# Ham3798/shielded-pool-pinocchio-solana

Measured on AMD Instinct MI355X. Metric: Groth16 proofs/sec, higher is better.
Workload: dtype u32x8 (254-bit Montgomery integers); 1 GPU; audit_circuit (RLWE, const-PK; scripts/generate_audit.py:246-465), batch of 2048 independent proofs per GPU per step, every row a distinct witness; circuit=audit, n_constraints=29178, n_wires=35432, domain=32768, batch_per_gpu=2048, n_distinct_witnesses=2048, table_bytes=223485100032, parallelism=independent proofs x1, pk_bytes=9850060

## Files before the change

shielded-pool-pinocchio-solana_amd/csrc/kernels.hpp:

```cpp
#pragma once
#include <hip/hip_runtime.h>
#include <stdint.h>
#include "bn254.hpp"
#include "msm_plan.hpp"
#include "rlwe_ntt.hpp"

namespace spp {

struct DevSparse {
  const uint32_t* rowptr;
  const uint32_t* wire;
  const uint32_t* coeff;
  const uint32_t* lit;
};
static constexpr uint32_t COEFF_ONE = 0x80000000u;
static constexpr uint32_t COEFF_MINUS_ONE = 0x40000000u;
static constexpr uint32_t COEFF_MASK = 0x3fffffffu;

struct DevCircuit {
  DevSparse A, B, C, H;
  const Fr* coeffs;
  const Fr* aux;
  const uint32_t* program;
  uint32_t n_wires, n_constraints, n_public, n_inputs, challenge_wire;
  const uint32_t* run_start;
  uint32_t n_runs;
  uint32_t max_row_terms;
  const uint8_t* row_flags;
  const uint32_t* sm_wires;
  const int32_t* sm_lo;
  uint32_t sm_nslots;
  const uint32_t* sm_rowptr;
  const uint32_t* sm_slot;
  const int32_t* sm_coef;
  const uint32_t* sm_rest_ptr;
  const uint32_t* sm_rest_wire;
  const uint32_t* sm_rest_coeff;
  const uint32_t* sm_row_out;
  uint32_t sm_nrows;
  const uint8_t* row_small;
  const uint32_t* lg_rows;
  uint32_t lg_n;
  const uint8_t* row_long;
  const Fr* pos3_rc;  const Fr* pos3_mds;
  const Fr* pos5_rc;  const Fr* pos5_mds;
  const Fr* p2_rc;    const Fr* p2_mu;
  const Fr* byte_mont;
  const uint32_t* pos3_mds29;
  const uint32_t* pos5_mds29;
};

struct HashConsts {
  const Fr* pos3_rc;  const Fr* pos3_mds;
  const Fr* pos5_rc;  const Fr* pos5_mds;
  const Fr* p2_rc;    const Fr* p2_mu;
  const uint32_t* pos3_mds29;
  const uint32_t* pos5_mds29;
};

struct RlwePkDev {
  int32_t hat[2][2][1024];
  uint32_t nzeros[2];
  uint16_t zeros[2][1024];
};
struct RlweDev {
  RnTables tb;
  int32_t pk_scale[2];
  RlwePkDev* pk = nullptr;
};
void launch_rlwe_witness(hipStream_t st, const RlweDev& rd, const uint32_t* pk_a, const uint32_t* pk_b, const int8_t* r, const int8_t* e1,
                         const int8_t* e2, const uint8_t* msg, uint32_t* c0, uint32_t* c1, int32_t* k0, int32_t* k1, uint8_t* packed_be,
                         uint32_t count);
void launch_poseidon_hash(hipStream_t st, HashConsts hc, const uint8_t* in_be, uint32_t arity, uint8_t* out_be, uint32_t count);
void launch_merkle_path(hipStream_t st, HashConsts hc, const uint8_t* leaf_be, const uint64_t* index, const uint8_t* siblings_be,
                        uint32_t depth, uint8_t* root_be, uint32_t count);
void launch_merkle_level(hipStream_t st, HashConsts hc, const Fr* children, uint32_t n_children, Fr dflt, Fr* parents, uint32_t n_parents);
struct MerkleTreeDev {
  Fr* level[33];
  uint64_t count[33];
  Fr dflt[33];
  uint32_t depth;
};
void launch_merkle_defaults(hipStream_t st, HashConsts hc, Fr* out, uint32_t depth);
void launch_merkle_update(hipStream_t st, HashConsts hc, const Fr* children, uint64_t n_children, const Fr* dflt_level, Fr* parents,
                          uint64_t first, uint32_t n);
void launch_merkle_gather(hipStream_t st, const MerkleTreeDev* t, uint32_t depth, const uint64_t* indices, uint32_t nq, uint8_t* out_be);
void launch_fr_from_be(hipStream_t st, const uint8_t* in, Fr* out, uint32_t n);
void launch_fr_to_be(hipStream_t st, const Fr* in, uint8_t* out, uint32_t n);
void launch_grumpkin_keygen(hipStream_t st, const GkAffine* table, const uint8_t* sk_be, uint8_t* xy_be, uint32_t count);
void launch_withdraw_rows(hipStream_t st, const GkAffine* table, HashConsts hc, const MerkleTreeDev* t, const uint8_t* notes, uint8_t* rows,
                          uint32_t count);
void launch_deposit_leaves(hipStream_t st, const GkAffine* table, HashConsts hc, const uint8_t* deposits, Fr* leaves, uint32_t count);
void launch_deposit_roots(hipStream_t st, HashConsts hc, const MerkleTreeDev* t, uint64_t first, uint32_t count, uint8_t* roots_be,
                          uint8_t* commitments_be);
void launch_poseidon2_sponge(hipStream_t st, HashConsts hc, const uint8_t* in_be, uint32_t n, uint8_t* out_be, uint32_t count);
void launch_rlwe_decrypt(hipStream_t st, const uint32_t* sk_mod_q, const uint32_t* c0, const uint32_t* c1, uint8_t* msg, uint32_t count);
void launch_shamir_combine(hipStream_t st, const Fr* lambda, const uint8_t* ys_be, uint32_t t, uint32_t n, uint8_t* secret_be,
                           uint32_t* sk_mod_q);
void launch_audit_msg(hipStream_t st, const uint8_t* xy_be, uint8_t* msg, uint32_t count);
void launch_audit_assemble(hipStream_t st, const uint8_t* wa_be, const uint8_t* ct_be, const uint8_t* packed_be, const uint8_t* sk_be,
                           const int8_t* r, const int8_t* e1, const int8_t* e2, const int32_t* k0, const int32_t* k1, uint8_t* rows,
                           uint32_t count);

void launch_load_inputs(hipStream_t st, const uint8_t* d_inputs_be, const uint8_t* d_rs_be, Fr* W, uint32_t n_inputs,
                        uint32_t n_wires, uint32_t P);
static constexpr uint32_t SOLVE_SCRATCH_MIN_ROWS = 324;
void launch_solve(hipStream_t st, DevCircuit dc, Fr* W, Fr* scratch, uint32_t pc_begin, uint32_t pc_end, uint32_t P);
enum : uint32_t { COOP_SEQ = 0, COOP_PAR = 1, COOP_LEVELS = 2, COOP_POSEIDON = 3, COOP_POSEIDON2 = 4, COOP_GRUMPKIN = 5, COOP_LEVEL_STREAM = 6 };
struct DevCoop {
  const uint32_t* items;
  const uint32_t* par;
  const uint32_t* lvl_ptr;
  const uint32_t* lvl_rows;
  const uint32_t* lvl_stream;
};
static constexpr uint32_t COOP_CHUNK = 1024;
static constexpr uint32_t COOP_TRACKS = 4;
struct CoopTracks { uint32_t n; uint32_t begin[COOP_TRACKS], end[COOP_TRACKS]; };
void launch_solve_coop(hipStream_t st, DevCircuit dc, DevCoop co, Fr* W, Fr* scratch, CoopTracks tracks, uint32_t P);
void launch_batch_div(hipStream_t st, DevCircuit dc, Fr* W, Fr* scratch, uint32_t k0, uint32_t n, uint32_t P);
void launch_count8(hipStream_t st, DevCircuit dc, Fr* W, uint32_t* counters, uint32_t h0, uint32_t n, uint32_t out0, uint32_t P);
struct VerifyKeyDev;
void launch_verify(hipStream_t st, const VerifyKeyDev* vk, const uint8_t* proofs, const uint8_t* pws, uint32_t pw_len, uint32_t count,
                   int32_t* ok);
struct PairingCheckDev;
void launch_pairing_check(hipStream_t st, const PairingCheckDev* a, int32_t* ok);
void launch_spmv_check(hipStream_t st, DevCircuit dc, const Fr* W, Fr* abc, uint32_t n, uint32_t P, uint32_t* status, int16_t* small = nullptr);

void launch_ntt(hipStream_t st, Fr* data, uint32_t logn, uint32_t P, const Fr* tw, bool dif, uint32_t nbatch, size_t batch_stride,
                const Fr* post = nullptr);
void launch_scale_rows(hipStream_t st, Fr* data, const Fr* table, uint32_t n, uint32_t P, uint32_t nbatch, size_t batch_stride);
void launch_qap_pointwise(hipStream_t st, Fr* abc, uint32_t n, uint32_t P, Fr zinv);
void launch_qap_product(hipStream_t st, Fr* abc, uint32_t n, uint32_t P);

template <class F>
struct MsmWalk;
template <>
struct MsmWalk<Fq> {
  static constexpr uint32_t waves_per_simd = 2;
  static constexpr bool gather_ahead = false;
};
template <>
struct MsmWalk<Fq2> {
  static constexpr uint32_t waves_per_simd = 1;
  static constexpr bool gather_ahead = true;
};
template <class F>
void launch_build_table(hipStream_t st, const Affine<F>* bases, uint32_t N, uint32_t c, uint32_t Wt, uint32_t row0, uint32_t nrows,
                        Affine<F>* table, XYZZ<F>* tmp, F* tmp_pre);
void launch_msm_digits(hipStream_t st, const uint32_t* rows, const Fr* scalars, int16_t* dig, uint32_t N, uint32_t P, uint32_t c);
template <class F>
void launch_msm_accumulate(hipStream_t st, const Affine<F>* table, const int16_t* dig, XYZZ<F>* partial, uint32_t N, uint32_t P, uint32_t c,
                           const MsmPlan& pl, hipEvent_t ev_start = nullptr, hipEvent_t ev_stop = nullptr);
template <class F>
void launch_msm_reduce(hipStream_t st, XYZZ<F>* partial, XYZZ<F>* out, uint32_t P, const MsmPlan& pl, uint32_t c, bool empty);
static constexpr uint32_t MSM_FOLD_SETS = 8;
static constexpr uint32_t MSM_FOLD_RADIX = 8;
template <class F>
struct MsmFoldSets {
  XYZZ<F>* partial[MSM_FOLD_SETS];
  XYZZ<F>* out[MSM_FOLD_SETS];
  uint32_t Sg[MSM_FOLD_SETS], R[MSM_FOLD_SETS], c[MSM_FOLD_SETS];
  uint32_t cur[MSM_FOLD_SETS], half[MSM_FOLD_SETS];
};
template <class F>
void launch_msm_reduce_multi(hipStream_t st, MsmFoldSets<F> fs, uint32_t nsets, uint32_t P);

void launch_g1_eval_basis(hipStream_t st, const G1Affine* pts, uint32_t n_pts, uint32_t logn, const Fr* scale, const Fr* tw_inv, G1XYZZ* work,
                          G1Affine* out);

void launch_g1_column_sums(hipStream_t st, const G1Affine* base, const uint32_t* row, const Fr* coeff, uint32_t nterms, const uint32_t* seg,
                           uint32_t nseg, G1XYZZ* work, G1Affine* out);

size_t pippenger_workspace_bytes(uint32_t n);
size_t pippenger_workspace_bytes_g2(uint32_t n);
void launch_pippenger_g2(hipStream_t st, const G2Affine* bases, const Fr* scalars, uint32_t n, void* workspace, G2XYZZ** out_windows,
                         hipEvent_t ev0, hipEvent_t ev1);
uint32_t pippenger_windows();
void launch_pippenger_g1(hipStream_t st, const G1Affine* bases, const Fr* scalars, uint32_t n, void* workspace, G1XYZZ** out_windows,
                         hipEvent_t ev0, hipEvent_t ev1);

void launch_challenge(hipStream_t st, const G1XYZZ* commit, Fr* W, uint32_t challenge_wire, uint32_t P, G1Affine* commit_affine,
                      uint32_t* status);
struct AssembleArgs {
  const G1XYZZ* mA; const G1XYZZ* mB1; const G2XYZZ* mB2; const G1XYZZ* mK; const G1XYZZ* mZ; const G1XYZZ* mPok;
  const G1Affine* commit_affine;
  const Fr* W; uint32_t row_r, row_s; uint32_t n_public;
  const G1XYZZ* sAr; const G1XYZZ* rBs1;
  uint8_t* proofs;
  uint8_t* pws;
  uint32_t P;
};
void launch_assemble(hipStream_t st, AssembleArgs a);
void launch_spin(hipStream_t st, uint64_t ticks_100mhz, uint32_t* sink);
void launch_touch(hipStream_t st, uint32_t* sink);
void launch_scale_witness(hipStream_t st, const Fr* W, Fr* Ws, Fr* Wr, uint32_t n_rows, uint32_t row_r, uint32_t row_s, uint32_t P);

template <class F>
void launch_fixed_base_mul(hipStream_t st, const Affine<F>* gen_table, uint32_t c, const Fr* scalars, uint32_t n, Affine<F>* out);

}
```

shielded-pool-pinocchio-solana_amd/csrc/kernels_msm.hip:

```cpp
#include "msm_table.hpp"

namespace spp {

template void launch_build_table<Fq>(hipStream_t, const Affine<Fq>*, uint32_t, uint32_t, uint32_t, uint32_t, uint32_t, Affine<Fq>*,
                                     XYZZ<Fq>*, Fq*);
template void launch_msm_accumulate<Fq>(hipStream_t, const Affine<Fq>*, const int16_t*, XYZZ<Fq>*, uint32_t, uint32_t, uint32_t, const MsmPlan&,
                                        hipEvent_t, hipEvent_t);
template void launch_msm_reduce_multi<Fq>(hipStream_t, MsmFoldSets<Fq>, uint32_t, uint32_t);
template void launch_msm_reduce<Fq>(hipStream_t, XYZZ<Fq>*, XYZZ<Fq>*, uint32_t, const MsmPlan&, uint32_t, bool);
template void launch_fixed_base_mul<Fq>(hipStream_t, const Affine<Fq>*, uint32_t, const Fr*, uint32_t, Affine<Fq>*);

__global__ void __launch_bounds__(256) k_msm_digits(const uint32_t* __restrict__ rows, const Fr* __restrict__ scalars,
                                                    int16_t* __restrict__ dig, uint32_t N, uint32_t P, uint32_t Pp, uint32_t c, uint32_t W) {
  const uint64_t g = (uint64_t)blockIdx.x * blockDim.x + threadIdx.x;
  const uint32_t p = (uint32_t)(g % Pp), i = (uint32_t)(g / Pp);
  if (i >= N || p >= P) return;
  const Fr s = scalars[(size_t)rows[i] * P + p];
  uint32_t l[8];
  s.to_canonical(l);
  const bool neg = canonical_gt_half<FrParams>(l);
  if (neg) {
    uint32_t t[8];
    canonical_negate<FrParams>(l, t);
    SPP_UNROLL for (int k = 0; k < 8; k++) l[k] = t[k];
  }
  const uint32_t mask = (1u << c) - 1u, half = 1u << (c - 1);
  uint32_t carry = 0;
  int16_t* out = dig + (size_t)i * Pp + p;
  const size_t plane = (size_t)N * Pp;
#pragma unroll 1
  for (uint32_t j = 0; j < W; j++) {
    const uint32_t d = (l[0] & mask) + carry;
    SPP_UNROLL for (int k = 0; k < 7; k++) l[k] = (l[k] >> c) | (l[k + 1] << (32 - c));
    l[7] >>= c;
    const bool over = neg ? d > half : d >= half;
    int v = over ? (int)d - (int)(1u << c) : (int)d;
    carry = over ? 1u : 0u;
    if (neg) v = -v;
    out[(size_t)j * plane] = (int16_t)v;
  }
}
void launch_msm_digits(hipStream_t st, const uint32_t* rows, const Fr* scalars, int16_t* dig, uint32_t N, uint32_t P, uint32_t c) {
  if (N == 0 || P == 0) return;
  const uint32_t Pp = msm_padded_batch(P);
  const uint64_t lanes = (uint64_t)N * Pp;
  hipLaunchKernelGGL(k_msm_digits, dim3((uint32_t)((lanes + 255) / 256)), dim3(256), 0, st, rows, scalars, dig, N, P, Pp, c, msm_windows(c));
}

__device__ __forceinline__ XYZZ<Fq> g1_scalar_mul(const XYZZ<Fq>& pt, const Fr& k) {
  uint32_t c[8];
  k.to_canonical(c);
  XYZZ<Fq> acc = XYZZ<Fq>::infinity();
  if (pt.is_inf()) return acc;
#pragma unroll 1
  for (int w = 7; w >= 0; w--) {
    const uint32_t word = w == 0 ? c[0] : w == 1 ? c[1] : w == 2 ? c[2] : w == 3 ? c[3] : w == 4 ? c[4] : w == 5 ? c[5] : w == 6 ? c[6] : c[7];
#pragma unroll 1
    for (int bit = 31; bit >= 0; bit--) {
      acc.dbl_inplace();
      if ((word >> bit) & 1) acc.add(pt);
    }
  }
  return acc;
}
__global__ void __launch_bounds__(64) k_g1_dft_load(const G1Affine* __restrict__ pts, uint32_t n_pts, const Fr* __restrict__ scale,
                                                    G1XYZZ* __restrict__ x, uint32_t n) {
  const uint32_t j = blockIdx.x * blockDim.x + threadIdx.x;
  if (j >= n) return;
  x[j] = j < n_pts ? g1_scalar_mul(G1XYZZ::from_affine(pts[j]), scale[j]) : G1XYZZ::infinity();
}
__global__ void __launch_bounds__(64) k_g1_dft_stage(G1XYZZ* __restrict__ x, uint32_t n, uint32_t len, const Fr* __restrict__ tw) {
  const uint32_t g = blockIdx.x * blockDim.x + threadIdx.x;
  if (g >= n / 2) return;
  const uint32_t half = len / 2, j = g % half, b = (g / half) * len;
  G1XYZZ u = x[b + j], v = x[b + j + half];
  G1XYZZ d = u;
  d.add(v.neg());
  u.add(v);
  x[b + j] = u;
  const uint32_t e = j * (n / len);
  x[b + j + half] = e ? g1_scalar_mul(d, tw[e]) : d;
}
__global__ void __launch_bounds__(64) k_g1_to_affine(const G1XYZZ* __restrict__ x, G1Affine* __restrict__ out, uint32_t n) {
  const uint32_t i = blockIdx.x * blockDim.x + threadIdx.x;
  if (i < n) out[i] = x[i].to_affine();
}
__global__ void __launch_bounds__(64) k_g1_terms(const G1Affine* __restrict__ base, const uint32_t* __restrict__ row, const Fr* __restrict__ coeff,
                                                 uint32_t nterms, G1XYZZ* __restrict__ out) {
  const uint32_t t = blockIdx.x * blockDim.x + threadIdx.x;
  if (t >= nterms) return;
  const G1XYZZ p = G1XYZZ::from_affine(base[row[t]]);
  const Fr c = coeff[t];
  if (c == Fr::one()) out[t] = p;
  else if (c == Fr::one().neg()) out[t] = p.neg();
  else out[t] = g1_scalar_mul(p, c);
}
__global__ void __launch_bounds__(64) k_g1_segsum(const G1XYZZ* __restrict__ terms, const uint32_t* __restrict__ seg, uint32_t nseg,
                                                  G1Affine* __restrict__ out) {
  const uint32_t s = blockIdx.x * blockDim.x + threadIdx.x;
  if (s >= nseg) return;
  G1XYZZ acc = G1XYZZ::infinity();
  for (uint32_t t = seg[s]; t < seg[s + 1]; t++) acc.add(terms[t]);
  out[s] = acc.to_affine();
}
void launch_g1_column_sums(hipStream_t st, const G1Affine* base, const uint32_t* row, const Fr* coeff, uint32_t nterms, const uint32_t* seg,
                           uint32_t nseg, G1XYZZ* work, G1Affine* out) {
  if (nterms) hipLaunchKernelGGL(k_g1_terms, dim3((nterms + 63) / 64), dim3(64), 0, st, base, row, coeff, nterms, work);
  if (nseg) hipLaunchKernelGGL(k_g1_segsum, dim3((nseg + 63) / 64), dim3(64), 0, st, work, seg, nseg, out);
}
void launch_g1_eval_basis(hipStream_t st, const G1Affine* pts, uint32_t n_pts, uint32_t logn, const Fr* scale, const Fr* tw_inv, G1XYZZ* work,
                          G1Affine* out) {
  const uint32_t n = 1u << logn;
  hipLaunchKernelGGL(k_g1_dft_load, dim3((n + 63) / 64), dim3(64), 0, st, pts, n_pts, scale, work, n);
  for (uint32_t len = n; len >= 2; len >>= 1)
    hipLaunchKernelGGL(k_g1_dft_stage, dim3((n / 2 + 63) / 64), dim3(64), 0, st, work, n, len, tw_inv);
  hipLaunchKernelGGL(k_g1_to_affine, dim3((n + 63) / 64), dim3(64), 0, st, work, out, n);
}

}
```

shielded-pool-pinocchio-solana_amd/csrc/kernels_msm_g2.hip:

```cpp
#include "msm_table.hpp"

namespace spp {

template void launch_build_table<Fq2>(hipStream_t, const Affine<Fq2>*, uint32_t, uint32_t, uint32_t, uint32_t, uint32_t, Affine<Fq2>*,
                                      XYZZ<Fq2>*, Fq2*);
template void launch_msm_accumulate<Fq2>(hipStream_t, const Affine<Fq2>*, const int16_t*, XYZZ<Fq2>*, uint32_t, uint32_t, uint32_t,
                                         const MsmPlan&, hipEvent_t, hipEvent_t);
template void launch_msm_reduce_multi<Fq2>(hipStream_t, MsmFoldSets<Fq2>, uint32_t, uint32_t);
template void launch_msm_reduce<Fq2>(hipStream_t, XYZZ<Fq2>*, XYZZ<Fq2>*, uint32_t, const MsmPlan&, uint32_t, bool);
template void launch_fixed_base_mul<Fq2>(hipStream_t, const Affine<Fq2>*, uint32_t, const Fr*, uint32_t, Affine<Fq2>*);

}
```

shielded-pool-pinocchio-solana_amd/csrc/msm_table.hpp:

```cpp
#pragma once
#include <hip/hip_ext.h>
#include "kernels.hpp"
#include <algorithm>
#include "f29.hpp"

namespace spp {

static constexpr unsigned MSM_FOLD_COOP_MAX_BATCH = 8;
static constexpr unsigned MSM_WALK_BLOCK = 64;

template <class F>
__global__ void __launch_bounds__(64) k_build_table(const Affine<F>* __restrict__ bases, uint32_t N, uint32_t c, uint32_t Wn,
                                                    uint32_t step_bits, uint32_t row0, uint32_t nrows, Affine<F>* __restrict__ table,
                                                    XYZZ<F>* __restrict__ tmp, F* __restrict__ tmp_pre) {
  const uint32_t rl = blockIdx.x * blockDim.x + threadIdx.x;
  if (rl >= nrows) return;
  const uint32_t row = row0 + rl;
  const uint32_t E = 1u << (c - 1);
  Affine<F>* out = table + ((size_t)(row >> 6) * E) * 64 + (row & 63);
  XYZZ<F>* t = tmp + rl;
  F* pre = tmp_pre + rl;
  if (row >= N * Wn) {
    for (uint32_t d = 0; d < E; d++) out[(size_t)d * 64] = Affine<F>::infinity();
    return;
  }
  const uint32_t i = row / Wn, j = row % Wn;
  Affine<F> base = bases[i];
  if (base.is_inf()) {
    for (uint32_t d = 0; d < E; d++) out[(size_t)d * 64] = Affine<F>::infinity();
    return;
  }
  XYZZ<F> b = XYZZ<F>::from_affine(base);
  for (uint32_t k = 0; k < step_bits * j; k++) b.dbl_inplace();
  Affine<F> bj = b.to_affine();
  XYZZ<F> acc = XYZZ<F>::from_affine(bj);
  F prod = F::one();
  for (uint32_t d = 0; d < E; d++) {
    t[(size_t)d * nrows] = acc;
    pre[(size_t)d * nrows] = prod;
    prod = prod * (acc.ZZ * acc.ZZZ);
    acc.madd(bj);
  }
  F inv = prod.inv();
  for (uint32_t d = E; d-- > 0;) {
    XYZZ<F> q = t[(size_t)d * nrows];
    F I = inv * pre[(size_t)d * nrows];
    inv = inv * (q.ZZ * q.ZZZ);
    F izz = I * q.ZZZ;
    F izzz = I * q.ZZ;
    out[(size_t)d * 64] = {q.X * izz, q.Y * izzz};
  }
}
template <class F>
void launch_build_table(hipStream_t st, const Affine<F>* bases, uint32_t N, uint32_t c, uint32_t Wt, uint32_t row0, uint32_t nrows,
                        Affine<F>* table, XYZZ<F>* tmp, F* tmp_pre) {
  if (nrows == 0) return;
  const uint32_t W = msm_windows(c);
  if (Wt == 0 || Wt > W) Wt = W;
  const uint32_t R = (W + Wt - 1) / Wt;
  hipLaunchKernelGGL(k_build_table<F>, dim3((nrows + 63) / 64), dim3(64), 0, st, bases, N, c, Wt, c * R, row0, nrows, table, tmp, tmp_pre);
}

struct Recoder {
  uint32_t l[8];
  uint32_t carry;
  bool neg;
  __device__ __forceinline__ void init(const Fr& s) {
    uint32_t cl[8];
    s.to_canonical(cl);
    neg = canonical_gt_half<FrParams>(cl);
    if (neg) {
      canonical_negate<FrParams>(cl, l);
    } else {
      SPP_UNROLL for (int k = 0; k < 8; k++) l[k] = cl[k];
    }
    carry = 0;
  }
  __device__ __forceinline__ uint32_t next(uint32_t c, bool& sgn) {
    const uint32_t mask = (1u << c) - 1u, half = 1u << (c - 1);
    uint32_t d = (l[0] & mask) + carry;
    SPP_UNROLL for (int k = 0; k < 7; k++) l[k] = (l[k] >> c) | (l[k + 1] << (32 - c));
    l[7] >>= c;
    if (d > half) {
      d = (1u << c) - d;
      carry = 1;
      sgn = !neg;
    } else {
      carry = 0;
      sgn = neg;
    }
    return d;
  }
};

__device__ __forceinline__ bool words_all_zero(const Fq& v) {
  uint32_t o = 0;
  SPP_UNROLL for (int i = 0; i < 8; i++) o |= v.l[i];
  return o == 0;
}
template <class F>
struct MsmAcc;
template <>
struct MsmAcc<Fq> {
  XYZZ29<FqParams> a;
  __device__ __forceinline__ void init() { a = XYZZ29<FqParams>::infinity(); }
  __device__ __forceinline__ void madd(const Affine<Fq>& e, bool sgn) {
    if (words_all_zero(e.x) && words_all_zero(e.y)) return;
    a.madd(e, sgn);
  }
  __device__ __forceinline__ XYZZ<Fq> result() const { return a.to_xyzz(); }
};

template <>
struct MsmAcc<Fq2> {
  XYZZ29G2 a;
  __device__ __forceinline__ void init() { a = XYZZ29G2::infinity(); }
  __device__ __forceinline__ void madd(const Affine<Fq2>& e, bool sgn) {
    if (words_all_zero(e.x.c0) && words_all_zero(e.x.c1) && words_all_zero(e.y.c0) && words_all_zero(e.y.c1)) return;
    a.madd(e, sgn);
  }
  __device__ __forceinline__ XYZZ<Fq2> result() const { return a.to_xyzz(); }
};


template <class F>
__global__ void __launch_bounds__(MSM_WALK_BLOCK, MsmWalk<F>::waves_per_simd) k_msm_flat(const Affine<F>* __restrict__ table, const int16_t* __restrict__ dig,
                                                  XYZZ<F>* __restrict__ partial, uint32_t N, uint32_t P, uint32_t Pp, uint32_t c,
                                                  uint32_t R, uint32_t Sg) {
  const uint32_t g = blockIdx.x * blockDim.x + threadIdx.x;
  const uint32_t p = g % Pp, t = g / Pp;
  if (t >= R * Sg || p >= P) return;
  const uint32_t rho = t / Sg, sl = t % Sg;
  const uint32_t E = 1u << (c - 1);
  const int16_t* __restrict__ dg = dig + ((size_t)rho * N) * Pp + p;
  MsmAcc<F> acc;
  acc.init();
  if constexpr (MsmWalk<F>::gather_ahead) {
    int d_next = 0;
    Affine<F> e_next;
    for (uint32_t i0 = sl;; i0 += 4 * Sg) {
      const bool last = i0 >= N;
      uint64_t pack = 0;
      if (!last) {
        SPP_UNROLL for (uint32_t k = 0; k < 4; k++) {
          const uint32_t i = i0 + k * Sg;
          const uint32_t d = i < N ? (uint32_t)(uint16_t)dg[(size_t)i * Pp] : 0u;
          pack |= (uint64_t)d << (16 * k);
        }
      }
#pragma unroll 1
      for (uint32_t k = 0; k < 4; k++) {
        const int d = (int)(int16_t)(uint16_t)(pack >> (16 * k));
        const bool flush = last && k == 0;
        if (d != 0 || flush) {
          Affine<F> e;
          if (d != 0) {
            const uint32_t i = i0 + k * Sg;
            const uint32_t mag = (uint32_t)(d < 0 ? -d : d);
            e = table[((size_t)(i >> 6) * E + (mag - 1)) * 64 + (i & 63)];
          }
          if (d_next != 0) acc.madd(e_next, d_next < 0);
          d_next = d;
          if (d != 0) e_next = e;
        }
      }
      if (last) break;
    }
  } else {
    for (uint32_t i0 = sl; i0 < N; i0 += 4 * Sg) {
      uint64_t pack = 0;
      SPP_UNROLL for (uint32_t k = 0; k < 4; k++) {
        const uint32_t i = i0 + k * Sg;
        const uint32_t d = i < N ? (uint32_t)(uint16_t)dg[(size_t)i * Pp] : 0u;
        pack |= (uint64_t)d << (16 * k);
      }
      if (pack == 0) continue;
#pragma unroll 1
      for (uint32_t k = 0; k < 4; k++) {
        const int d = (int)(int16_t)(uint16_t)(pack >> (16 * k));
        if (d != 0) {
          const uint32_t i = i0 + k * Sg;
          const uint32_t mag = (uint32_t)(d < 0 ? -d : d);
          acc.madd(table[((size_t)(i >> 6) * E + (mag - 1)) * 64 + (i & 63)], d < 0);
        }
      }
    }
  }
  partial[(size_t)t * P + p] = acc.result();
}

template <class F>
__global__ void __launch_bounds__(256) k_msm_rows(const Affine<F>* __restrict__ table, const int16_t* __restrict__ dig,
                                                  XYZZ<F>* __restrict__ partial, uint32_t N, uint32_t P, uint32_t Pp, uint32_t c,
                                                  uint32_t Wt, uint32_t R, uint32_t W, uint32_t Sg, uint32_t Q, uint32_t Wq) {
  const uint32_t g = blockIdx.x * blockDim.x + threadIdx.x;
  const uint32_t p = g % Pp, t = g / Pp;
  if (t >= R * Sg || p >= P) return;
  const uint32_t rho = t / Sg, sl = t % Sg;
  const uint32_t E = 1u << (c - 1);
  const size_t plane = (size_t)N * Pp;
  MsmAcc<F> acc;
  acc.init();
  const uint32_t items = N * Q;
  for (uint32_t it = sl; it < items; it += Sg) {
    uint32_t i = it, q = 0;
    if (Q > 1) {
      i = it % N;
      q = it / N;
    }
    const uint32_t m0 = q * Wq, m1 = m0 + Wq < Wt ? m0 + Wq : Wt;
    const int16_t* __restrict__ dg = dig + (size_t)i * Pp + p;
#pragma unroll 1
    for (uint32_t m = m0; m < m1; m++) {
      const uint32_t j = rho + R * m;
      if (j >= W) break;
      const int d = dg[(size_t)j * plane];
      if (d != 0) {
        const uint32_t row = i * Wt + m;
        const uint32_t mag = (uint32_t)(d < 0 ? -d : d);
        acc.madd(table[((size_t)(row >> 6) * E + (mag - 1)) * 64 + (row & 63)], d < 0);
      }
    }
  }
  partial[(size_t)t * P + p] = acc.result();
}

template <class F>
void launch_msm_accumulate(hipStream_t st, const Affine<F>* table, const int16_t* dig, XYZZ<F>* partial, uint32_t N, uint32_t P, uint32_t c,
                           const MsmPlan& pl, hipEvent_t ev_start, hipEvent_t ev_stop) {
  if (N == 0 || P == 0) {
    if (ev_start) hipEventRecord(ev_start, st);
    if (ev_stop) hipEventRecord(ev_stop, st);
    return;
  }
  const uint64_t lanes = (uint64_t)pl.R * pl.Sg * pl.Pp;
  if (pl.Wt == 1)
    hipExtLaunchKernelGGL(k_msm_flat<F>, dim3((uint32_t)((lanes + MSM_WALK_BLOCK - 1) / MSM_WALK_BLOCK)), dim3(MSM_WALK_BLOCK), 0, st, ev_start, ev_stop, 0, table, dig, partial, N, P, pl.Pp, c, pl.R, pl.Sg);
  else
    hipExtLaunchKernelGGL(k_msm_rows<F>, dim3((uint32_t)((lanes + 255) / 256)), dim3(256), 0, st, ev_start, ev_stop, 0, table, dig, partial, N, P, pl.Pp, c,
                          pl.Wt, pl.R, pl.W, pl.Sg, pl.Q, pl.Wq);
}

template <class T>
__device__ __forceinline__ T msm_shfl_xor(const T& v, int mask) {
  static_assert(sizeof(T) % 4 == 0, "word-sized");
  T r;
  const uint32_t* s = reinterpret_cast<const uint32_t*>(&v);
  uint32_t* d = reinterpret_cast<uint32_t*>(&r);
  SPP_UNROLL for (uint32_t i = 0; i < sizeof(T) / 4; i++) d[i] = (uint32_t)__shfl_xor((int)s[i], mask, 64);
  return r;
}
template <class F>
__global__ void __launch_bounds__(64) k_msm_fold_multi(MsmFoldSets<F> fs, uint32_t P, uint32_t coop) {
  const uint32_t set = blockIdx.y, rho = blockIdx.z;
  const uint32_t next = fs.half[set], S_cur = fs.cur[set];
  if (next == 0 || rho >= fs.R[set]) return;
  const uint32_t g = blockIdx.x * blockDim.x + threadIdx.x;
  XYZZ<F>* __restrict__ partial = fs.partial[set] + (size_t)rho * fs.Sg[set] * P;
  if (coop) {
    static_assert(MSM_FOLD_RADIX == 8, "three shuffle steps");
    const uint32_t o = g >> 3, m = g & 7;
    const bool live = o < next * P;
    const uint32_t s = live ? o / P : 0, p = live ? o % P : 0, t = s + next * m;
    XYZZ<F> a = XYZZ<F>::infinity();
    if (live && t < S_cur) a = partial[(size_t)t * P + p];
    SPP_UNROLL for (int d = 4; d >= 1; d >>= 1) {
      const XYZZ<F> b = msm_shfl_xor(a, d);
      a.add(b);
    }
    if (live && m == 0) {
      if (next == 1 && fs.R[set] == 1) fs.out[set][p] = a;
      else partial[(size_t)s * P + p] = a;
    }
    return;
  }
  if (g >= next * P) return;
  const uint32_t s = g / P, p = g % P;
  XYZZ<F> a = partial[(size_t)s * P + p];
#pragma unroll 1
  for (uint32_t t = s + next; t < S_cur; t += next) a.add(partial[(size_t)t * P + p]);
  if (next == 1 && fs.R[set] == 1) fs.out[set][p] = a;
  else partial[(size_t)s * P + p] = a;
}
template <class F>
__global__ void __launch_bounds__(64) k_msm_horner(MsmFoldSets<F> fs, uint32_t P) {
  const uint32_t set = blockIdx.y;
  const uint32_t R = fs.R[set], c = fs.c[set];
  const uint32_t p = blockIdx.x * blockDim.x + threadIdx.x;
  if (R <= 1 || p >= P) return;
  const size_t stride = (size_t)fs.Sg[set] * P;
  const XYZZ<F>* __restrict__ sums = fs.partial[set];
  XYZZ<F> acc = sums[(size_t)(R - 1) * stride + p];
#pragma unroll 1
  for (uint32_t rho = R - 1; rho-- > 0;) {
    if (!acc.is_inf()) {
      F X = acc.X * acc.ZZ, Y = acc.Y * acc.ZZZ, Z = acc.ZZ;
#pragma unroll 1
      for (uint32_t k = 0; k < c; k++) {
        const F A = X.sqr(), B = Y.sqr(), C = B.sqr();
        const F t = (X + B).sqr() - A - C;
        const F D = t.dbl();
        const F E = A.dbl() + A;
        const F X3 = E.sqr() - D.dbl();
        const F C8 = C.dbl().dbl().dbl();
        const F Z3 = (Y * Z).dbl();
        Y = E * (D - X3) - C8;
        X = X3;
        Z = Z3;
      }
      const F zz = Z.sqr();
      acc.X = X;
      acc.Y = Y;
      acc.ZZ = zz;
      acc.ZZZ = zz * Z;
    }
    acc.add(sums[(size_t)rho * stride + p]);
  }
  fs.out[set][p] = acc;
}
template <class F>
__global__ void __launch_bounds__(256) k_msm_fill_inf(XYZZ<F>* __restrict__ out, uint32_t P) {
  const uint32_t g = blockIdx.x * blockDim.x + threadIdx.x;
  if (g < P) out[g] = XYZZ<F>::infinity();
}

template <class F>
void launch_msm_reduce_multi(hipStream_t st, MsmFoldSets<F> fs, uint32_t nsets, uint32_t P) {
  if (P == 0 || nsets == 0) return;
  uint32_t cur[MSM_FOLD_SETS];
  bool done[MSM_FOLD_SETS];
  uint32_t maxR = 1;
  bool horner = false;
  for (uint32_t i = 0; i < nsets; i++) {
    cur[i] = fs.Sg[i];
    done[i] = false;
    if (fs.Sg[i] == 0) {
      hipLaunchKernelGGL(k_msm_fill_inf<F>, dim3((P + 255) / 256), dim3(256), 0, st, fs.out[i], P);
      done[i] = true;
      fs.R[i] = 1;
      continue;
    }
    if (fs.R[i] > 1) horner = true;
    if (fs.R[i] > 1 && fs.Sg[i] == 1) done[i] = true;
    maxR = std::max(maxR, fs.R[i]);
  }
  for (;;) {
    uint64_t lanes = 0;
    for (uint32_t i = 0; i < nsets; i++) {
      fs.half[i] = done[i] ? 0 : (cur[i] + MSM_FOLD_RADIX - 1) / MSM_FOLD_RADIX;
      fs.cur[i] = cur[i];
      lanes = std::max<uint64_t>(lanes, (uint64_t)fs.half[i] * P);
    }
    if (lanes == 0) break;
    const uint32_t coop = P <= MSM_FOLD_COOP_MAX_BATCH ? 1u : 0u;
    if (coop) lanes *= MSM_FOLD_RADIX;
    hipLaunchKernelGGL(k_msm_fold_multi<F>, dim3((uint32_t)((lanes + 63) / 64), nsets, maxR), dim3(64), 0, st, fs, P, coop);
    for (uint32_t i = 0; i < nsets; i++)
      if (!done[i]) {
        cur[i] = fs.half[i];
        if (cur[i] == 1) done[i] = true;
      }
  }
  if (horner) {
    for (uint32_t i = 0; i < nsets; i++)
      if (fs.Sg[i] == 0) fs.R[i] = 1;
    hipLaunchKernelGGL(k_msm_horner<F>, dim3((P + 63) / 64, nsets), dim3(64), 0, st, fs, P);
  }
}
template <class F>
void launch_msm_reduce(hipStream_t st, XYZZ<F>* partial, XYZZ<F>* out, uint32_t P, const MsmPlan& pl, uint32_t c, bool empty) {
  MsmFoldSets<F> fs{};
  fs.partial[0] = partial;
  fs.out[0] = out;
  fs.Sg[0] = empty ? 0 : pl.Sg;
  fs.R[0] = pl.R;
  fs.c[0] = c;
  launch_msm_reduce_multi<F>(st, fs, 1, P);
}

template <class F>
__global__ void __launch_bounds__(64) k_fixed_base_mul(const Affine<F>* __restrict__ gen_table, uint32_t c, uint32_t Wn,
                                                       const Fr* __restrict__ scalars, uint32_t n, Affine<F>* __restrict__ out) {
  const uint32_t i = blockIdx.x * blockDim.x + threadIdx.x;
  if (i >= n) return;
  const uint32_t E = 1u << (c - 1);
  Fr s = scalars[i];
  XYZZ<F> acc = XYZZ<F>::infinity();
  if (!s.is_zero()) {
    Recoder rc;
    rc.init(s);
#pragma unroll 1
    for (uint32_t j = 0; j < Wn; j++) {
      bool sgn;
      uint32_t d = rc.next(c, sgn);
      if (d != 0) {
        Affine<F> e = gen_table[((size_t)(j >> 6) * E + (d - 1)) * 64 + (j & 63)];
        if (sgn) e.y = e.y.neg();
        acc.madd(e);
      }
    }
  }
  out[i] = acc.to_affine();
}
template <class F>
void launch_fixed_base_mul(hipStream_t st, const Affine<F>* gen_table, uint32_t c, const Fr* scalars, uint32_t n, Affine<F>* out) {
  if (n == 0) return;
  hipLaunchKernelGGL(k_fixed_base_mul<F>, dim3((n + 63) / 64), dim3(64), 0, st, gen_table, c, msm_windows(c), scalars, n, out);
}

}
```

shielded-pool-pinocchio-solana_amd/csrc/spp_circuit.hpp:

```cpp
#pragma once
#include "spp_internal.hpp"

template <class F>
struct MsmSet {
  uint32_t N = 0;
  Affine<F>* table = nullptr;
  uint32_t* rows = nullptr;
  bool from_h = false;
  uint32_t c = 0;
  uint32_t Wt = 0;
};
template <class F>
struct MsmBuf {
  XYZZ<F>* partial = nullptr;
  XYZZ<F>* out = nullptr;
  size_t partial_cap = 0;
  MsmPlan plan{};
};
struct Workspace {
  hipStream_t st = nullptr;
  hipStream_t st2 = nullptr;
  hipStream_t own_st = nullptr, own_st2 = nullptr;
  hipStream_t own_st2p = nullptr;
  std::pair<hipEvent_t, hipEvent_t> g2_ev{nullptr, nullptr};
  hipEvent_t ev_w = nullptr, ev_b2 = nullptr;
  hipEvent_t ev_in = nullptr, ev_rows = nullptr;
  size_t cap = 0, last_P = 0;
  Fr *W = nullptr, *abc = nullptr, *scratch = nullptr;
  G1Affine* commit_affine = nullptr;
  uint8_t *d_inputs = nullptr, *d_rs = nullptr, *d_proofs = nullptr, *d_pws = nullptr;
  uint32_t* d_status = nullptr;
  uint32_t* counters = nullptr;
  MsmBuf<Fq> A, B1, K, Z, CB, CS;
  MsmBuf<Fq> sA, rB;
  Fr *Ws = nullptr, *Wr = nullptr;
  MsmBuf<Fq2> B2;
  int16_t *dig1 = nullptr, *dig2 = nullptr;
  size_t dig1_cap = 0, dig2_cap = 0;
  int16_t* small = nullptr;
  void* audit_scratch = nullptr;
  size_t audit_scratch_cap = 0;
  std::vector<void*> owned;
  hipEvent_t ev[8] = {};
  std::vector<std::pair<hipEvent_t, hipEvent_t>> msm_ev;
  size_t msm_ev_used = 0;
};

template <class F>
struct PendingTable {
  std::vector<Affine<F>> pts;
  Affine<F>* table;
  uint32_t c, Wt;
};
struct SolveStep {
  enum Kind { SEQ, BATCH_DIV, COUNT8, COMMIT } kind;
  uint32_t a = 0, b = 0, c = 0;
  uint32_t ntracks = 0, tr_begin[COOP_TRACKS] = {}, tr_end[COOP_TRACKS] = {};
};
struct Switches {
  int h_mode = 2;
  bool no_coop = false;
  bool trace_items = false;
  bool one_track = false;
  bool no_level_stream = false;
  uint32_t coop_max_batch = 1024;
  bool no_side = false;
  int forced_depth = 0;
  bool no_split = false;
  MsmTuning msm;
};
static constexpr uint64_t SCALED_BLIND_MAX_SCALARS = 1500000;
inline uint32_t scaled_blind_max_batch(uint32_t n_a, uint32_t n_b1) {
  const uint64_t n = (uint64_t)n_a + n_b1;
  return n ? (uint32_t)std::max<uint64_t>(1, std::min<uint64_t>(1024, SCALED_BLIND_MAX_SCALARS / n)) : 1;
}
struct spp_circuit {
  spp_ctx* ctx = nullptr;
  std::vector<SolveStep> schedule;
  Circuit circ;
  DevCircuit dc{};
  uint32_t c_bits = 10, n = 0, logn = 0;
  uint32_t max_batch_div = SOLVE_SCRATCH_MIN_ROWS;
  DevCoop coop{};
  Switches sw;
  bool generic_solver = false;
  uint32_t row_r = 0, row_s = 0, row_rs = 0, n_rows = 0;
  size_t in_stride = 0, pw_stride = 0;
  uint64_t table_bytes = 0;
  MsmSet<Fq> A, B1, K, Z, CB, CS;
  MsmSet<Fq2> B2;
  Fr *tw_fwd = nullptr, *tw_inv = nullptr, *coset_br = nullptr, *coset_inv_br = nullptr;
  Fr zinv;
  std::vector<void*> owned;
  Workspace ws[SPP_NWS];
  int next_ws = 0, last_ws = 0, prev_ws = 0;
  std::vector<PendingTable<Fq>> pending1;
  std::vector<PendingTable<Fq2>> pending2;
};

template <class T>
static int own_upload(spp_circuit* c, T** dst, const std::vector<T>& src) {
  HIP_TRY(dev_upload(dst, src));
  c->owned.push_back((void*)*dst);
  return 0;
}

#pragma GCC visibility push(hidden)
int coop_plan(spp_circuit* c);
int row_paths_plan(spp_circuit* c);
void destroy_circuit(spp_circuit* c);
void free_workspace(Workspace& w);
#pragma GCC visibility pop
```

shielded-pool-pinocchio-solana_amd/csrc/spp_load.cpp:

```cpp
#include "spp_circuit.hpp"

static std::vector<PendingTable<Fq>>& pending(spp_circuit* c, Fq*) { return c->pending1; }
static std::vector<PendingTable<Fq2>>& pending(spp_circuit* c, Fq2*) { return c->pending2; }

static int upload_sparse(spp_circuit* c, const Circuit& circ, const Sparse& m, DevSparse* out) {
  std::vector<uint32_t> wire(m.terms.size()), coeff(m.terms.size()), lit(m.terms.size(), 0);
  Fr one = Fr::one(), mone = Fr::one().neg();
  std::vector<uint32_t> small(circ.coeffs.size(), 0);
  for (size_t ci = 0; ci < circ.coeffs.size(); ci++) {
    uint32_t v[8], nv[8];
    circ.coeffs[ci].to_canonical(v);
    bool hi0 = true;
    for (int k = 1; k < 8; k++) hi0 = hi0 && v[k] == 0;
    if (hi0 && v[0] != 0 && v[0] < (1u << 28)) { small[ci] = v[0]; continue; }
    circ.coeffs[ci].neg().to_canonical(nv);
    hi0 = true;
    for (int k = 1; k < 8; k++) hi0 = hi0 && nv[k] == 0;
    if (hi0 && nv[0] != 0 && nv[0] < (1u << 28)) small[ci] = nv[0] | 0x80000000u;
  }
  for (size_t i = 0; i < m.terms.size(); i++) {
    wire[i] = m.terms[i].wire;
    uint32_t ci = m.terms[i].coeff;
    uint32_t flag = 0;
    if (circ.coeffs[ci] == one) flag = COEFF_ONE;
    else if (circ.coeffs[ci] == mone) flag = COEFF_MINUS_ONE;
    else lit[i] = small[ci];
    coeff[i] = ci | flag;
  }
  uint32_t *rp, *w, *co, *li;
  if (int e = own_upload(c, &li, lit)) return e;
  out->lit = li;
  if (int e = own_upload(c, &rp, m.rowptr)) return e;
  if (int e = own_upload(c, &w, wire)) return e;
  if (int e = own_upload(c, &co, coeff)) return e;
  out->rowptr = rp;
  out->wire = w;
  out->coeff = co;
  return 0;
}

template <class F>
static int alloc_table(spp_circuit* c, size_t N, uint32_t cbits, uint32_t Wt, Affine<F>** table_out) {
  size_t table_elems = std::max<size_t>(msm_table_elems((uint32_t)N, cbits, Wt), 1);
  Affine<F>* table;
  HIP_TRY(hipMalloc((void**)&table, table_elems * sizeof(Affine<F>)));
  c->owned.push_back(table);
  c->table_bytes += table_elems * sizeof(Affine<F>);
  *table_out = table;
  return 0;
}
template <class F>
static int build_table(spp_circuit* c, const std::vector<Affine<F>>& pts, uint32_t cbits, uint32_t Wt, Affine<F>* table, size_t temp_budget) {
  hipStream_t st = c->ctx->stream;
  const uint32_t Wn = Wt, E = 1u << (cbits - 1);
  const size_t N = pts.size();
  if (N == 0) return 0;
  const size_t rows_total = msm_table_rows(N, Wn);
  const size_t per_row = (size_t)E * (sizeof(XYZZ<F>) + sizeof(F));
  size_t chunk = std::max<size_t>(64, ((temp_budget / per_row) / 64) * 64);
  chunk = std::min(chunk, (size_t)65536);
  chunk = std::min(chunk, rows_total);
  DevBuf d_bases, tmp, tmp_pre;
  HIP_TRY(d_bases.alloc(N * sizeof(Affine<F>)));
  HIP_TRY(hipMemcpy(d_bases.p, pts.data(), N * sizeof(Affine<F>), hipMemcpyHostToDevice));
  HIP_TRY(tmp.alloc(chunk * E * sizeof(XYZZ<F>)));
  HIP_TRY(tmp_pre.alloc(chunk * E * sizeof(F)));
  for (size_t r0 = 0; r0 < rows_total; r0 += chunk) {
    uint32_t cnt = (uint32_t)std::min(chunk, rows_total - r0);
    launch_build_table<F>(st, d_bases.as<Affine<F>>(), (uint32_t)N, cbits, Wt, (uint32_t)r0, cnt, table, tmp.as<XYZZ<F>>(), tmp_pre.as<F>());
  }
  HIP_TRY(hipStreamSynchronize(st));
  HIP_TRY(hipGetLastError());
  return 0;
}
static size_t table_temp_budget() {
  size_t free_b = 0, total_b = 0;
  if (hipMemGetInfo(&free_b, &total_b) != hipSuccess) return (size_t)2 << 30;
  size_t b = free_b / 2;
  b = std::min(b, (size_t)48 << 30);
  return std::max(b, (size_t)1 << 28);
}
template <class F>
static int build_table_chunked(spp_circuit* c, const std::vector<Affine<F>>& pts, uint32_t cbits, uint32_t Wt, Affine<F>** table_out) {
  if (int e = alloc_table<F>(c, pts.size(), cbits, Wt, table_out)) return e;
  return build_table<F>(c, pts, cbits, Wt, *table_out, std::min(table_temp_budget(), (size_t)2 << 30));
}


template <class F>
static int make_set(spp_circuit* c, MsmSet<F>* set, const std::vector<uint32_t>& rows, const std::vector<Affine<F>>& pts, bool from_h,
                    uint32_t cbits, bool flat) {
  set->N = (uint32_t)pts.size();
  set->from_h = from_h;
  set->c = cbits;
  set->Wt = flat ? 1 : msm_windows(cbits);
  if (int e = own_upload(c, &set->rows, rows)) return e;
  if (int e = alloc_table<F>(c, pts.size(), cbits, set->Wt, &set->table)) return e;
  pending(c, (F*)nullptr).push_back({pts, set->table, cbits, set->Wt});
  return 0;
}
static int build_pending(spp_circuit* c) {
  const size_t budget = table_temp_budget();
  int e = 0;
  for (auto& p : pending(c, (Fq*)nullptr)) if (!e) e = build_table<Fq>(c, p.pts, p.c, p.Wt, p.table, budget);
  for (auto& p : pending(c, (Fq2*)nullptr)) if (!e) e = build_table<Fq2>(c, p.pts, p.c, p.Wt, p.table, budget);
  pending(c, (Fq*)nullptr).clear();
  pending(c, (Fq2*)nullptr).clear();
  return e;
}

namespace {
struct PkFile {
  uint32_t circuit_id, n_wires, domain_log, n_public, challenge_wire;
  G1Affine alpha1, beta1, delta1;
  G2Affine beta2, delta2;
  std::vector<uint32_t> A_w, B1_w, B2_w, K_w, CB_w, CS_w;
  std::vector<G1Affine> A, B1, K, Z, CB, CS;
  std::vector<G2Affine> B2;
};
struct Rd {
  const uint8_t* p;
  const uint8_t* end;
  bool ok = true;
  uint32_t u32() {
    if (p + 4 > end) { ok = false; return 0; }
    uint32_t v = (uint32_t)p[0] | ((uint32_t)p[1] << 8) | ((uint32_t)p[2] << 16) | ((uint32_t)p[3] << 24);
    p += 4;
    return v;
  }
  const uint8_t* take(size_t n) {
    if (p + n > end) { ok = false; return nullptr; }
    const uint8_t* q = p;
    p += n;
    return q;
  }
};
bool rd_g1_section(Rd& r, std::vector<uint32_t>* wires, std::vector<G1Affine>& pts) {
  uint32_t n = r.u32();
  if (!r.ok || (size_t)n * 64 > (size_t)(r.end - r.p)) return false;
  if (wires) {
    wires->resize(n);
    for (auto& w : *wires) w = r.u32();
  }
  pts.resize(n);
  for (auto& pt : pts) {
    const uint8_t* b = r.take(64);
    if (!b) return false;
    pt = g1_from_raw(b);
  }
  return r.ok;
}
bool parse_pk(const std::vector<uint8_t>& buf, PkFile& k) {
  Rd r{buf.data(), buf.data() + buf.size()};
  if (r.u32() != 0x4b505053u || r.u32() != 1) return false;
  k.circuit_id = r.u32(); k.n_wires = r.u32(); k.domain_log = r.u32(); k.n_public = r.u32(); k.challenge_wire = r.u32();
  const uint8_t* b;
  if (!(b = r.take(64))) return false; k.alpha1 = g1_from_raw(b);
  if (!(b = r.take(64))) return false; k.beta1 = g1_from_raw(b);
  if (!(b = r.take(64))) return false; k.delta1 = g1_from_raw(b);
  if (!(b = r.take(128))) return false; k.beta2 = g2_from_raw(b);
  if (!(b = r.take(128))) return false; k.delta2 = g2_from_raw(b);
  if (!rd_g1_section(r, &k.A_w, k.A)) return false;
  if (!rd_g1_section(r, &k.B1_w, k.B1)) return false;
  uint32_t n2 = r.u32();
  if (!r.ok || (size_t)n2 * 128 > (size_t)(r.end - r.p)) return false;
  k.B2_w.resize(n2);
  for (auto& w : k.B2_w) w = r.u32();
  k.B2.resize(n2);
  for (auto& pt : k.B2) {
    if (!(b = r.take(128))) return false;
    pt = g2_from_raw(b);
  }
  if (!rd_g1_section(r, &k.K_w, k.K)) return false;
  if (!rd_g1_section(r, nullptr, k.Z)) return false;
  if (!rd_g1_section(r, &k.CB_w, k.CB)) return false;
  if (!rd_g1_section(r, &k.CS_w, k.CS)) return false;
  return r.ok && r.p == r.end;
}
}


template <class F>
static void merge_point(std::vector<uint32_t>& wires, std::vector<Affine<F>>& pts, uint32_t wire, const Affine<F>& extra) {
  for (size_t i = 0; i < wires.size(); i++)
    if (wires[i] == wire) {
      pts[i] = host_add(pts[i], extra);
      return;
    }
  wires.push_back(wire);
  pts.push_back(extra);
}

namespace {
struct PlanSet {
  double n, esz, wgt;
  bool flat;
  int bits;
};
double plan_bytes(const PlanSet& s, int cb) { return s.n * s.esz * (s.flat ? 1.0 : (double)msm_windows((uint32_t)cb)) * (double)(1u << (cb - 1)); }
void plan_greedy(std::vector<PlanSet>& sets, double budget, int cmax) {
  double used = 0;
  for (auto& s : sets) used += plan_bytes(s, s.bits);
  for (;;) {
    int best = -1;
    double best_gain = 0;
    for (size_t i = 0; i < sets.size(); i++) {
      const PlanSet& s = sets[i];
      if (s.wgt == 0 || s.bits >= cmax || s.n == 0) continue;
      const double extra = plan_bytes(s, s.bits + 1) - plan_bytes(s, s.bits);
      if (used + extra > budget) continue;
      const double saved = s.wgt * s.n * ((double)msm_windows((uint32_t)s.bits) - (double)msm_windows((uint32_t)s.bits + 1));
      double gain = saved / extra;
      if (saved <= 0) gain = 1e-30;
      if (gain > best_gain) { best_gain = gain; best = (int)i; }
    }
    if (best < 0) break;
    used += plan_bytes(sets[best], sets[best].bits + 1) - plan_bytes(sets[best], sets[best].bits);
    sets[best].bits++;
  }
}
const double PLAN_ESZ[7] = {64, 64, 64, 64, 64, 64, 128}, PLAN_WGT[7] = {1, 1, 1, 1, 0, 0, 3.0};
}

struct LoadState {
  PkFile pk;
  uint32_t cw[7];
  bool flat[7] = {false, false, false, false, false, false, false};
  std::vector<uint32_t> z_w, xk_w;
  std::vector<G1Affine> z_p, xk_p;
};

static Switches read_switches() {
  Switches sw;
  const char* hm = getenv("SPP_H_MODE");
  sw.h_mode = hm ? atoi(hm) : (getenv("SPP_Z_COEFF") ? 0 : 2);
  if (sw.h_mode < 0 || sw.h_mode > 2) sw.h_mode = 2;
  sw.no_coop = getenv("SPP_NO_COOP") != nullptr;
  sw.trace_items = getenv("SPP_COOP_TRACE") != nullptr;
  sw.one_track = getenv("SPP_COOP_ONE_TRACK") != nullptr;
  sw.no_level_stream = getenv("SPP_NO_LEVEL_STREAM") != nullptr;
  if (const char* e = getenv("SPP_COOP_MAX")) sw.coop_max_batch = (uint32_t)atoi(e);
  sw.no_side = getenv("SPP_NO_SIDE") != nullptr;
  const char* de = getenv("SPP_DEPTH");
  const int depth = de ? atoi(de) : 0;
  sw.forced_depth = depth >= 1 && depth <= SPP_NWS ? depth : 0;
  sw.no_split = getenv("SPP_NO_SPLIT") != nullptr;
  sw.msm = msm_tuning_from_env(getenv("SPP_MSM_WAVES"), getenv("SPP_MSM_WAVES_SMALL"));
  return sw;
}

static int plan_load_windows(const PkFile& pk, int window_bits, const uint32_t* forced_bits, uint32_t cw[7], bool flat[7]) {
  const double nset[7] = {(double)pk.A.size() + 2, (double)pk.B1.size() + 2, (double)pk.K.size() + 1, (double)pk.Z.size(),
                          (double)pk.CB.size(), (double)pk.CS.size(), (double)pk.B2.size() + 2};
  if (forced_bits) {
    for (int s = 0; s < 7; s++) {
      cw[s] = forced_bits[s];
      flat[s] = PLAN_WGT[s] != 0;
    }
  } else if (window_bits != 0) {
    for (int s = 0; s < 7; s++) cw[s] = (uint32_t)window_bits;
  } else {
    const char* fe = getenv("SPP_FLAT");
    const bool use_flat = !(fe && fe[0] == '0');
    size_t free_b = 0, total_b = 0;
    HIP_TRY(hipMemGetInfo(&free_b, &total_b));
    double budget = 240e9;
    if (const char* env = getenv("SPP_TABLE_BUDGET_GB")) budget = atof(env) * 1e9;
    budget = std::min(budget, 0.85 * (double)free_b);
    std::vector<PlanSet> sets;
    for (int s = 0; s < 7; s++) {
      flat[s] = use_flat && PLAN_WGT[s] != 0;
      sets.push_back({nset[s], PLAN_ESZ[s], PLAN_WGT[s], flat[s], PLAN_WGT[s] != 0 ? 6 : 9});
    }
    plan_greedy(sets, budget, use_flat ? 16 : 15);
    for (int s = 0; s < 7; s++) cw[s] = (uint32_t)sets[s].bits;
  }
  return 0;
}

static int load_r1cs(spp_circuit* c) {
  const Circuit& circ = c->circ;
  int e;
  if ((e = upload_sparse(c, circ, circ.A, &c->dc.A)) || (e = upload_sparse(c, circ, circ.B, &c->dc.B)) ||
      (e = upload_sparse(c, circ, circ.C, &c->dc.C)) || (e = upload_sparse(c, circ, circ.H, &c->dc.H)))
    return e;
  Fr* d_coeffs;
  Fr* d_aux;
  uint32_t* d_prog;
  if ((e = own_upload(c, &d_coeffs, circ.coeffs)) || (e = own_upload(c, &d_prog, circ.program)) || (e = own_upload(c, &d_aux, circ.aux))) return e;
  c->dc.coeffs = d_coeffs;
  c->dc.aux = d_aux;
  c->dc.program = d_prog;
  c->dc.n_wires = circ.n_wires;
  c->dc.n_constraints = circ.n_constraints;
  {
    std::vector<uint32_t> runs;
    auto same_b = [&](uint32_t k) {
      const uint32_t a0 = circ.B.rowptr[k - 1], a1 = circ.B.rowptr[k], b1 = circ.B.rowptr[k + 1];
      if (a1 - a0 != b1 - a1 || a1 == a0) return false;
      for (uint32_t t = 0; t < a1 - a0; t++)
        if (circ.B.terms[a0 + t].wire != circ.B.terms[a1 + t].wire || circ.B.terms[a0 + t].coeff != circ.B.terms[a1 + t].coeff) return false;
      return true;
    };
    uint32_t len = 0;
    for (uint32_t k = 0; k < circ.n_constraints; k++) {
      if (k == 0 || len >= 8 || !same_b(k)) { runs.push_back(k); len = 0; }
      len++;
    }
    const uint32_t n_runs = (uint32_t)runs.size();
    runs.push_back(circ.n_constraints);
    uint32_t* d_runs;
    if ((e = own_upload(c, &d_runs, runs))) return e;
    c->dc.run_start = d_runs;
    c->dc.n_runs = n_runs;
    uint32_t longest = 0;
    for (const Sparse* m : {&circ.A, &circ.B, &circ.C})
      for (uint32_t k = 0; k < circ.n_constraints; k++) longest = std::max(longest, m->rowptr[k + 1] - m->rowptr[k]);
    c->dc.max_row_terms = longest;
    std::vector<uint8_t> flags(std::max<uint32_t>(circ.n_constraints, 1), 0);
    for (uint32_t k = 0; k < circ.n_constraints; k++) {
      if (k > 0 && same_b(k)) flags[k] |= 1;
      const uint32_t a0 = circ.A.rowptr[k], a1 = circ.A.rowptr[k + 1], b0 = circ.B.rowptr[k], b1 = circ.B.rowptr[k + 1];
      bool eq = a1 - a0 == b1 - b0 && a1 != a0;
      for (uint32_t t = 0; eq && t < a1 - a0; t++)
        eq = circ.A.terms[a0 + t].wire == circ.B.terms[b0 + t].wire && circ.A.terms[a0 + t].coeff == circ.B.terms[b0 + t].coeff;
      if (eq) flags[k] |= 2;
    }
    uint8_t* d_flags;
    if ((e = own_upload(c, &d_flags, flags))) return e;
    c->dc.row_flags = d_flags;
  }
  c->dc.n_public = circ.n_public;
  c->dc.n_inputs = circ.n_inputs();
  c->dc.challenge_wire = circ.challenge_wire;
  {
    auto flat = [](const PoseidonParams& pp) {
      std::vector<Fr> m;
      for (auto& row : pp.mds)
        for (auto& v : row) m.push_back(v);
      return m;
    };
    const PoseidonParams& p3 = poseidon_params(3);
    const PoseidonParams& p5 = poseidon_params(5);
    const Poseidon2Params& p2 = poseidon2_params();
    Fr *a, *b, *cc, *d, *f, *g;
    std::vector<Fr> mu(p2.mu, p2.mu + 4);
    auto canon = [](std::vector<Fr> v) {
      for (auto& x : v) x = x.canonical();
      return v;
    };
    if ((e = own_upload(c, &a, canon(p3.rc))) || (e = own_upload(c, &b, flat(p3))) || (e = own_upload(c, &cc, canon(p5.rc))) ||
        (e = own_upload(c, &d, flat(p5))) || (e = own_upload(c, &f, p2.rc)) || (e = own_upload(c, &g, mu)))
      return e;
    std::vector<Fr> bytes(256);
    for (int i = 0; i < 256; i++) bytes[i] = Fr::from_u64((uint64_t)i);
    Fr* bm;
    if ((e = own_upload(c, &bm, bytes))) return e;
    c->dc.byte_mont = bm;
    auto flat29 = [](const PoseidonParams& pp) {
      std::vector<uint32_t> m;
      for (auto& row : pp.mds)
        for (auto& v : row) {
          const F29<FrParams> x = F29<FrParams>::from_fp(v);
          for (int k = 0; k < 9; k++) m.push_back(x.l[k]);
        }
      return m;
    };
    uint32_t *m3, *m5;
    if ((e = own_upload(c, &m3, flat29(p3))) || (e = own_upload(c, &m5, flat29(p5)))) return e;
    c->dc.pos3_mds29 = m3;
    c->dc.pos5_mds29 = m5;
    c->dc.pos3_rc = a; c->dc.pos3_mds = b; c->dc.pos5_rc = cc; c->dc.pos5_mds = d; c->dc.p2_rc = f; c->dc.p2_mu = g;
  }
  return 0;
}

static int load_program(spp_circuit* c) {
  const Circuit& circ = c->circ;
  bool generic_ops = false;
  {
    const auto& pr = circ.program;
    size_t pc = 0, seg = 0;
    auto flush = [&](size_t end) {
      if (end > seg) c->schedule.push_back({SolveStep::SEQ, (uint32_t)seg, (uint32_t)end, 0});
    };
    const bool trace_ops = getenv("SPP_SOLVE_TRACE") != nullptr;
    if (trace_ops) c->sw.no_coop = true;
    uint32_t prev_op = OP_END;
    while (pc < pr.size() && pr[pc] != OP_END) {
      if (trace_ops && pr[pc] != prev_op) {
        flush(pc);
        seg = std::max(seg, pc);
      }
      prev_op = pr[pc];
      switch (pr[pc]) {
        case OP_SOLVE_C: case OP_SOLVE_A: case OP_MASK: pc += 2; break;
        case OP_BATCH_DIV:
          c->max_batch_div = std::max(c->max_batch_div, pr[pc + 2]);
          if (pr[pc + 2] >= 64) {
            flush(pc);
            c->schedule.push_back({SolveStep::BATCH_DIV, pr[pc + 1], pr[pc + 2], 0});
            seg = pc + 3;
          }
          pc += 3;
          break;
        case OP_COUNT8:
          flush(pc);
          c->schedule.push_back({SolveStep::COUNT8, pr[pc + 1], pr[pc + 2], pr[pc + 3]});
          seg = pc + 4;
          pc += 4;
          break;
        case OP_BITS: case OP_LIMBS8: case OP_POSEIDON: pc += 4; break;
        case OP_POSEIDON2: case OP_INV_H: pc += 3; break;
        case OP_COMMIT:
          flush(pc);
          c->schedule.push_back({SolveStep::COMMIT, 0, 0, 0});
          pc += 1;
          seg = pc;
          break;
        case OP_GRUMPKIN: pc += 5 + pr[pc + 4]; break;
        case OP_SOLVE_ROW: case OP_LIMBS: case OP_COUNTN: pc += 5; generic_ops = true; break;
        case OP_GK_MUL: pc += 7; generic_ops = true; break;
        case OP_GLV: pc += 3 + 28; generic_ops = true; break;
        case OP_EMUL: pc += 3 + 16; generic_ops = true; break;
        default: return fail(SPP_ERR_FORMAT, "bad opcode %u in solver program", pr[pc]);
      }
    }
    flush(pc);
  }

  c->generic_solver = generic_ops;
  if (generic_ops) c->sw.no_coop = true;
  else if (int e = coop_plan(c)) return e;
  if (int e = row_paths_plan(c)) return e;
  return 0;
}

static int load_ntt_tables(spp_circuit* c) {
  int e;
  const uint32_t n = c->n, logn = c->logn;
  Fr w = fr_root_of_unity(logn), wi = w.inv();
  std::vector<Fr> tf(n / 2), ti(n / 2), cb(n), cib(n);
  Fr a = Fr::one(), b = Fr::one();
  for (uint32_t k = 0; k < n / 2; k++) {
    tf[k] = a;
    ti[k] = b;
    a = a * w;
    b = b * wi;
  }
  Fr g = c->sw.h_mode == 2 ? fr_root_of_unity(logn + 1) : Fr::from_u64(5), gi = g.inv(), ninv = Fr::from_u64(n).inv();
  std::vector<Fr> gp(n), gip(n);
  Fr x = ninv, y = ninv;
  for (uint32_t i = 0; i < n; i++) {
    gp[i] = x;
    gip[i] = y;
    x = x * g;
    y = y * gi;
  }
  for (uint32_t pos = 0; pos < n; pos++) {
    uint32_t i = bitrev(pos, logn);
    cb[pos] = gp[i];
    cib[pos] = gip[i];
  }
  if ((e = own_upload(c, &c->tw_fwd, tf)) || (e = own_upload(c, &c->tw_inv, ti)) || (e = own_upload(c, &c->coset_br, cb)) ||
      (e = own_upload(c, &c->coset_inv_br, cib)))
    return e;
  Fr gn = g.pow_u64(n);
  c->zinv = (gn - Fr::one()).inv();
  return 0;
}

static int load_key_sets(spp_circuit* c, const LoadState& s) {
  const PkFile& pk = s.pk;
  const uint32_t* cw = s.cw;
  const bool* flat = s.flat;
  int e;
  {
    std::vector<uint32_t> w = pk.A_w;
    std::vector<G1Affine> p = pk.A;
    merge_point(w, p, 0u, pk.alpha1);
    w.push_back(c->row_r); p.push_back(pk.delta1);
    if ((e = make_set(c, &c->A, w, p, false, cw[0], flat[0]))) return e;
  }
  {
    std::vector<uint32_t> w = pk.B1_w;
    std::vector<G1Affine> p = pk.B1;
    merge_point(w, p, 0u, pk.beta1);
    w.push_back(c->row_s); p.push_back(pk.delta1);
    if ((e = make_set(c, &c->B1, w, p, false, cw[1], flat[1]))) return e;
  }
  {
    std::vector<uint32_t> w = pk.B2_w;
    std::vector<G2Affine> p = pk.B2;
    merge_point(w, p, 0u, pk.beta2);
    w.push_back(c->row_s); p.push_back(pk.delta2);
    if ((e = make_set(c, &c->B2, w, p, false, cw[6], flat[6]))) return e;
  }
  return 0;
}

static int load_h_bases(spp_circuit* c, LoadState& s) {
  const PkFile& pk = s.pk;
  const Circuit& circ = c->circ;
  spp_ctx* ctx = c->ctx;
  std::vector<uint32_t>&z_w = s.z_w, &xk_w = s.xk_w;
  std::vector<G1Affine>&z_p = s.z_p, &xk_p = s.xk_p;
  int e;
  if (pk.Z.size() != (size_t)c->n - 1) return fail(SPP_ERR_FORMAT, "Z section has %zu points, expected %u", pk.Z.size(), c->n - 1);
  const uint32_t n = c->n;
  hipStream_t st = ctx->stream;
  auto eval_basis = [&](const std::vector<Fr>& scale, std::vector<G1Affine>& out) -> int {
    DevBuf d_pts, d_scale, d_work, d_out;
    HIP_TRY(d_pts.alloc(pk.Z.size() * sizeof(G1Affine)));
    HIP_TRY(d_scale.alloc((size_t)n * sizeof(Fr)));
    HIP_TRY(d_work.alloc((size_t)n * sizeof(G1XYZZ)));
    HIP_TRY(d_out.alloc((size_t)n * sizeof(G1Affine)));
    HIP_TRY(hipMemcpyAsync(d_pts.p, pk.Z.data(), pk.Z.size() * sizeof(G1Affine), hipMemcpyHostToDevice, st));
    HIP_TRY(hipMemcpyAsync(d_scale.p, scale.data(), (size_t)n * sizeof(Fr), hipMemcpyHostToDevice, st));
    launch_g1_eval_basis(st, d_pts.as<G1Affine>(), (uint32_t)pk.Z.size(), c->logn, d_scale.as<Fr>(), c->tw_inv, d_work.as<G1XYZZ>(),
                         d_out.as<G1Affine>());
    std::vector<G1Affine> br(n);
    HIP_TRY(hipMemcpyAsync(br.data(), d_out.p, (size_t)n * sizeof(G1Affine), hipMemcpyDeviceToHost, st));
    HIP_TRY(hipStreamSynchronize(st));
    HIP_TRY(hipGetLastError());
    out.resize(n);
    for (uint32_t pos = 0; pos < n; pos++) out[bitrev(pos, c->logn)] = br[pos];
    return 0;
  };
  if (c->sw.h_mode == 0) {
    for (uint32_t pos = 0; pos < n; pos++) {
      uint32_t i = bitrev(pos, c->logn);
      if (i == n - 1) continue;
      z_w.push_back(pos);
      z_p.push_back(pk.Z[i]);
    }
  } else if (c->sw.h_mode == 1) {
    Fr gi = Fr::from_u64(5).inv(), x = Fr::from_u64(n).inv();
    std::vector<Fr> scale(n);
    for (uint32_t j = 0; j < n; j++) { scale[j] = x; x = x * gi; }
    if ((e = eval_basis(scale, z_p))) return e;
    for (uint32_t i = 0; i < n; i++) z_w.push_back(i);
  } else {
    const Fr inv2n = Fr::from_u64(2 * (uint64_t)n).inv();
    std::vector<Fr> scale(n, inv2n);
    std::vector<G1Affine> WH;
    if ((e = eval_basis(scale, WH))) return e;
    Fr zi = fr_root_of_unity(c->logn + 1).inv(), x = inv2n.neg();
    for (uint32_t j = 0; j < n; j++) { scale[j] = x; x = x * zi; }
    if ((e = eval_basis(scale, z_p))) return e;
    for (uint32_t i = 0; i < n; i++) z_w.push_back(i);
    struct Tm { uint32_t wire, row; Fr cf; };
    std::vector<Tm> tms;
    for (uint32_t k = 0; k < circ.n_constraints; k++)
      for (uint32_t t = circ.C.rowptr[k]; t < circ.C.rowptr[k + 1]; t++) tms.push_back({circ.C.terms[t].wire, k, circ.coeffs[circ.C.terms[t].coeff]});
    std::stable_sort(tms.begin(), tms.end(), [](const Tm& a, const Tm& b) { return a.wire < b.wire; });
    std::vector<uint32_t> rows(tms.size()), seg{0};
    std::vector<Fr> cfs(tms.size());
    for (size_t t = 0; t < tms.size(); t++) {
      rows[t] = tms[t].row;
      cfs[t] = tms[t].cf;
      if (t + 1 == tms.size() || tms[t + 1].wire != tms[t].wire) {
        xk_w.push_back(tms[t].wire);
        seg.push_back((uint32_t)t + 1);
      }
    }
    if (!tms.empty()) {
      DevBuf d_base, d_rows, d_cfs, d_seg, d_work, d_out;
      HIP_TRY(d_base.alloc((size_t)n * sizeof(G1Affine)));
      HIP_TRY(d_rows.alloc(rows.size() * 4));
      HIP_TRY(d_cfs.alloc(cfs.size() * sizeof(Fr)));
      HIP_TRY(d_seg.alloc(seg.size() * 4));
      HIP_TRY(d_work.alloc(tms.size() * sizeof(G1XYZZ)));
      HIP_TRY(d_out.alloc(xk_w.size() * sizeof(G1Affine)));
      HIP_TRY(hipMemcpyAsync(d_base.p, WH.data(), (size_t)n * sizeof(G1Affine), hipMemcpyHostToDevice, st));
      HIP_TRY(hipMemcpyAsync(d_rows.p, rows.data(), rows.size() * 4, hipMemcpyHostToDevice, st));
      HIP_TRY(hipMemcpyAsync(d_cfs.p, cfs.data(), cfs.size() * sizeof(Fr), hipMemcpyHostToDevice, st));
      HIP_TRY(hipMemcpyAsync(d_seg.p, seg.data(), seg.size() * 4, hipMemcpyHostToDevice, st));
      launch_g1_column_sums(st, d_base.as<G1Affine>(), d_rows.as<uint32_t>(), d_cfs.as<Fr>(), (uint32_t)tms.size(), d_seg.as<uint32_t>(),
                            (uint32_t)xk_w.size(), d_work.as<G1XYZZ>(), d_out.as<G1Affine>());
      xk_p.resize(xk_w.size());
      HIP_TRY(hipMemcpyAsync(xk_p.data(), d_out.p, xk_p.size() * sizeof(G1Affine), hipMemcpyDeviceToHost, st));
      HIP_TRY(hipStreamSynchronize(st));
      HIP_TRY(hipGetLastError());
    }
  }
  return 0;
}

static int load_h_sets(spp_circuit* c, const LoadState& s) {
  const PkFile& pk = s.pk;
  const uint32_t* cw = s.cw;
  const bool* flat = s.flat;
  int e;
  const Circuit& circ = c->circ;
  const std::vector<uint32_t>&z_w = s.z_w, &xk_w = s.xk_w;
  const std::vector<G1Affine>&z_p = s.z_p, &xk_p = s.xk_p;
  {
    std::vector<uint32_t> w = pk.K_w;
    std::vector<G1Affine> p = pk.K;
    if (!xk_w.empty()) {
      std::vector<int32_t> at(circ.n_wires + 3, -1);
      for (size_t i = 0; i < w.size(); i++) at[w[i]] = (int32_t)i;
      for (size_t i = 0; i < xk_w.size(); i++) {
        if (xk_p[i].is_inf()) continue;
        if (at[xk_w[i]] >= 0) p[at[xk_w[i]]] = host_add(p[at[xk_w[i]]], xk_p[i]);
        else {
          at[xk_w[i]] = (int32_t)w.size();
          w.push_back(xk_w[i]);
          p.push_back(xk_p[i]);
        }
      }
    }
    w.push_back(c->row_rs); p.push_back(pk.delta1.neg());
    if ((e = make_set(c, &c->K, w, p, false, cw[2], flat[2]))) return e;
  }
  if ((e = make_set(c, &c->Z, z_w, z_p, true, cw[3], flat[3]))) return e;
  if ((e = make_set(c, &c->CB, pk.CB_w, pk.CB, false, cw[4], false))) return e;
  if ((e = make_set(c, &c->CS, pk.CS_w, pk.CS, false, cw[5], false))) return e;
  return build_pending(c);
}

static int load_streams(spp_circuit* c) {
  spp_ctx* ctx = c->ctx;
  for (int k = 0; k < SPP_NWS; k++) {
    Workspace& w = c->ws[k];
    const bool serial = getenv("SPP_SERIAL") != nullptr;
    w.own_st = ctx->pstream[k];
    if (int e = pick_concurrent_stream(w.own_st, &w.own_st2)) return e;
    {
      int lo = 0, hi = 0;
      HIP_TRY(hipDeviceGetStreamPriorityRange(&lo, &hi));
      const char* pe = getenv("SPP_ST2_PRIORITY");
      if (!(pe && pe[0] == '0') && hi < lo) HIP_TRY(hipStreamCreateWithPriority(&w.own_st2p, hipStreamDefault, hi));
    }
    w.st = serial ? ctx->pstream[0] : w.own_st;
    w.st2 = serial ? w.st : w.own_st2;
    HIP_TRY(hipEventCreate(&w.g2_ev.first));
    HIP_TRY(hipEventCreate(&w.g2_ev.second));
    HIP_TRY(hipEventCreateWithFlags(&w.ev_w, hipEventDisableTiming));
    HIP_TRY(hipEventCreateWithFlags(&w.ev_b2, hipEventDisableTiming));
    HIP_TRY(hipEventCreateWithFlags(&w.ev_in, hipEventDisableTiming));
    HIP_TRY(hipEventCreateWithFlags(&w.ev_rows, hipEventDisableTiming));
    HIP_TRY(hipEventRecord(w.ev_in, w.st));
    for (auto& evt : w.ev) HIP_TRY(hipEventCreate(&evt));
    w.msm_ev.resize(8);
    for (auto& pr : w.msm_ev) {
      HIP_TRY(hipEventCreate(&pr.first));
      HIP_TRY(hipEventCreate(&pr.second));
    }
  }
  return 0;
}

static int load_circuit_impl(spp_ctx* ctx, const char* circuit_path, const char* pk_path, int window_bits, const uint32_t* forced_bits,
                             spp_circuit** out) {
  if (!ctx || !circuit_path || !pk_path || !out) return fail(SPP_ERR_BAD_INPUT, "NULL argument");
  if (window_bits != 0 && (window_bits < 4 || window_bits > 16)) return fail(SPP_ERR_BAD_INPUT, "window_bits %d outside [4,16]", window_bits);
  std::lock_guard<std::mutex> lk(ctx->mu);
  HIP_TRY(hipSetDevice(ctx->device));
  spp_circuit* c = new spp_circuit();
  c->ctx = ctx;
  c->c_bits = (uint32_t)window_bits;
  struct Guard {
    spp_circuit* c;
    ~Guard() { if (c) destroy_circuit(c); }
  } guard{c};
  if (!c->circ.load(circuit_path)) return fail(SPP_ERR_IO, "cannot read circuit %s", circuit_path);
  std::vector<uint8_t> pkbuf;
  LoadState s;
  PkFile& pk = s.pk;
  if (!read_file(pk_path, pkbuf)) return fail(SPP_ERR_IO, "cannot read proving key %s", pk_path);
  if (!parse_pk(pkbuf, pk)) return fail(SPP_ERR_FORMAT, "malformed proving key %s", pk_path);
  const Circuit& circ = c->circ;
  if (pk.circuit_id != circ.id || pk.n_wires != circ.n_wires || pk.domain_log != circ.domain_log)
    return fail(SPP_ERR_FORMAT, "proving key does not match the circuit");
  c->sw = read_switches();
  if (int e = plan_load_windows(pk, window_bits, forced_bits, s.cw, s.flat)) return e;
  c->c_bits = s.cw[3];
  c->logn = circ.domain_log;
  c->n = 1u << c->logn;
  c->row_r = circ.n_wires;
  c->row_s = circ.n_wires + 1;
  c->row_rs = circ.n_wires + 2;
  c->n_rows = circ.n_wires + 3;
  c->in_stride = (size_t)circ.n_inputs() * 32;
  c->pw_stride = 12 + 32 * (size_t)(circ.n_public - 1);
  int e;
  if ((e = load_r1cs(c)) || (e = load_program(c)) || (e = load_ntt_tables(c)) || (e = load_key_sets(c, s)) || (e = load_h_bases(c, s)) ||
      (e = load_h_sets(c, s)) || (e = load_streams(c)))
    return e;
  guard.c = nullptr;
  *out = c;
  return SPP_OK;
}
extern "C" int spp_load_circuit(spp_ctx* ctx, const char* circuit_path, const char* pk_path, int window_bits, spp_circuit** out) {
  return load_circuit_impl(ctx, circuit_path, pk_path, window_bits, nullptr, out);
}
extern "C" int spp_load_circuit_with_windows(spp_ctx* ctx, const char* circuit_path, const char* pk_path, const uint32_t bits[7],
                                             spp_circuit** out) {
  if (!bits) return fail(SPP_ERR_BAD_INPUT, "NULL argument");
  for (int s = 0; s < 7; s++)
    if (bits[s] < 4 || bits[s] > 16) return fail(SPP_ERR_BAD_INPUT, "window bits %u of set %d outside [4,16]", bits[s], s);
  return load_circuit_impl(ctx, circuit_path, pk_path, 0, bits, out);
}

void free_workspace(Workspace& w) {
  if (w.audit_scratch) hipFree(w.audit_scratch);
  w.audit_scratch = nullptr;
  w.audit_scratch_cap = 0;
  for (void* p : w.owned) hipFree(p);
  w.owned.clear();
  w.cap = 0;
}
void destroy_circuit(spp_circuit* c) {
  if (!c) return;
  hipSetDevice(c->ctx->device);
  hipStreamSynchronize(c->ctx->stream);
  for (auto& w : c->ws) {
    if (w.st) hipStreamSynchronize(w.st);
    if (w.own_st2) { hipStreamSynchronize(w.own_st2); hipStreamDestroy(w.own_st2); }
    if (w.own_st2p) { hipStreamSynchronize(w.own_st2p); hipStreamDestroy(w.own_st2p); }
    if (w.g2_ev.first) hipEventDestroy(w.g2_ev.first);
    if (w.g2_ev.second) hipEventDestroy(w.g2_ev.second);
    if (w.ev_w) hipEventDestroy(w.ev_w);
    if (w.ev_b2) hipEventDestroy(w.ev_b2);
    if (w.ev_in) hipEventDestroy(w.ev_in);
    if (w.ev_rows) hipEventDestroy(w.ev_rows);
    free_workspace(w);
    for (auto& evt : w.ev) if (evt) hipEventDestroy(evt);
    for (auto& pr : w.msm_ev) {
      if (pr.first) hipEventDestroy(pr.first);
      if (pr.second) hipEventDestroy(pr.second);
    }
  }
  for (void* p : c->owned) hipFree(p);
  delete c;
}
extern "C" void spp_free_circuit(spp_circuit* c) { destroy_circuit(c); }
extern "C" int spp_circuit_info(const spp_circuit* c, uint32_t info[8]) {
  if (!c || !info) return fail(SPP_ERR_BAD_INPUT, "NULL argument");
  info[0] = c->circ.id; info[1] = c->circ.n_public - 1; info[2] = c->circ.n_secret; info[3] = c->circ.n_wires;
  info[4] = c->circ.n_constraints; info[5] = c->circ.domain_log; info[6] = c->circ.n_inputs(); info[7] = c->c_bits;
  return SPP_OK;
}
extern "C" uint64_t spp_circuit_table_bytes(const spp_circuit* c) { return c ? c->table_bytes : 0; }
extern "C" int spp_circuit_small_rows(const spp_circuit* c, uint32_t out[2]) {
  if (!c || !out) return fail(SPP_ERR_BAD_INPUT, "NULL argument");
  out[0] = c->dc.sm_nrows;
  out[1] = c->dc.sm_nslots;
  return SPP_OK;
}
extern "C" int spp_circuit_msm_windows(const spp_circuit* c, uint32_t bits[7]) {
  if (!c || !bits) return fail(SPP_ERR_BAD_INPUT, "NULL argument");
  bits[0] = c->A.c; bits[1] = c->B1.c; bits[2] = c->K.c; bits[3] = c->Z.c; bits[4] = c->CB.c; bits[5] = c->CS.c; bits[6] = c->B2.c;
  return SPP_OK;
}
extern "C" int spp_circuit_msm_table_rows(const spp_circuit* c, uint32_t rows[7]) {
  if (!c || !rows) return fail(SPP_ERR_BAD_INPUT, "NULL argument");
  rows[0] = c->A.Wt; rows[1] = c->B1.Wt; rows[2] = c->K.Wt; rows[3] = c->Z.Wt; rows[4] = c->CB.Wt; rows[5] = c->CS.Wt; rows[6] = c->B2.Wt;
  return SPP_OK;
}
extern "C" int spp_circuit_msm_sizes(const spp_circuit* c, uint32_t sizes[7]) {
  if (!c || !sizes) return fail(SPP_ERR_BAD_INPUT, "NULL argument");
  sizes[0] = c->A.N; sizes[1] = c->B1.N; sizes[2] = c->K.N; sizes[3] = c->Z.N; sizes[4] = c->CB.N; sizes[5] = c->CS.N; sizes[6] = c->B2.N;
  return SPP_OK;
}

extern "C" int spp_pk_msm_sizes(const char* pk_path, uint32_t sizes[7]) {
  if (!pk_path || !sizes) return fail(SPP_ERR_BAD_INPUT, "NULL argument");
  std::vector<uint8_t> pkbuf;
  PkFile pk;
  if (!read_file(pk_path, pkbuf)) return fail(SPP_ERR_IO, "cannot read proving key %s", pk_path);
  if (!parse_pk(pkbuf, pk)) return fail(SPP_ERR_FORMAT, "malformed proving key %s", pk_path);
  sizes[0] = (uint32_t)pk.A.size() + 2; sizes[1] = (uint32_t)pk.B1.size() + 2; sizes[2] = (uint32_t)pk.K.size() + 1;
  sizes[3] = (uint32_t)pk.Z.size(); sizes[4] = (uint32_t)pk.CB.size(); sizes[5] = (uint32_t)pk.CS.size(); sizes[6] = (uint32_t)pk.B2.size() + 2;
  return SPP_OK;
}
extern "C" int spp_plan_windows(uint32_t n_circuits, const uint32_t* sizes, double budget_bytes, uint32_t* bits) {
  if (!sizes || !bits || n_circuits == 0 || n_circuits > 16) return fail(SPP_ERR_BAD_INPUT, "bad argument");
  std::vector<PlanSet> sets;
  for (uint32_t k = 0; k < n_circuits; k++)
    for (int s = 0; s < 7; s++) sets.push_back({(double)sizes[7 * k + s], PLAN_ESZ[s], PLAN_WGT[s], PLAN_WGT[s] != 0, PLAN_WGT[s] != 0 ? 6 : 9});
  double floor_bytes = 0;
  for (auto& ps : sets) floor_bytes += plan_bytes(ps, ps.bits);
  if (floor_bytes > budget_bytes) return fail(SPP_ERR_BAD_INPUT, "the budget does not hold even 6-bit tables (%.1f GB needed)", floor_bytes / 1e9);
  plan_greedy(sets, budget_bytes, 16);
  for (size_t i = 0; i < sets.size(); i++) bits[i] = (uint32_t)sets[i].bits;
  return SPP_OK;
}
template <class F> static Affine<F> point_from_raw(const uint8_t* b);
template <> Affine<Fq> point_from_raw<Fq>(const uint8_t* b) { return g1_from_raw(b); }
template <> Affine<Fq2> point_from_raw<Fq2>(const uint8_t* b) { return g2_from_raw(b); }
static void point_to_raw(const G1Affine& p, uint8_t* b) { g1_to_raw(p, b); }
static void point_to_raw(const G2Affine& p, uint8_t* b) { g2_to_raw(p, b); }
template <class F, size_t PT_BYTES>
static int msm_fixed_unit(spp_ctx* ctx, const uint8_t* bases, const uint8_t* scalars, size_t n, int window_bits, uint8_t* out) {
  if (!ctx || !out || (n && (!bases || !scalars))) return fail(SPP_ERR_BAD_INPUT, "NULL argument");
  if (window_bits == 0) window_bits = 8;
  if (window_bits < 4 || window_bits > 16) return fail(SPP_ERR_BAD_INPUT, "window_bits outside [4,16]");
  std::lock_guard<std::mutex> lk(ctx->mu);
  HIP_TRY(hipSetDevice(ctx->device));
  hipStream_t st = ctx->stream;
  const uint32_t cb = (uint32_t)window_bits, Wn = msm_windows(cb);
  if ((uint64_t)msm_table_elems((uint32_t)n, cb, Wn) * PT_BYTES > ((uint64_t)64 << 30)) return fail(SPP_ERR_BAD_INPUT, "table would exceed 64 GiB; use a smaller window");
  std::vector<Affine<F>> pts(n);
  std::vector<Fr> sc(n);
  std::vector<uint32_t> rows(n);
  for (size_t i = 0; i < n; i++) {
    pts[i] = point_from_raw<F>(bases + PT_BYTES * i);
    sc[i] = Fr::from_bytes_be(scalars + 32 * i);
    rows[i] = (uint32_t)i;
  }
  spp_circuit tmpc;
  tmpc.ctx = ctx;
  tmpc.c_bits = cb;
  Affine<F>* table = nullptr;
  int e = build_table_chunked<F>(&tmpc, pts, cb, Wn, &table);
  Fr* d_sc = nullptr;
  uint32_t* d_rows = nullptr;
  XYZZ<F> *partial = nullptr, *d_out = nullptr;
  DevBuf dig;
  const MsmPlan pl = msm_plan((uint32_t)n, 1, cb, Wn, MsmWalk<F>::waves_per_simd, read_switches().msm);
  if (!e) e = own_upload(&tmpc, &d_sc, sc);
  if (!e) e = own_upload(&tmpc, &d_rows, rows);
  if (!e && hipMalloc((void**)&partial, sizeof(XYZZ<F>) * std::max<size_t>(pl.partial_elems(1), 1)) != hipSuccess) e = fail(SPP_ERR_HIP, "hipMalloc");
  if (!e && hipMalloc((void**)&d_out, sizeof(XYZZ<F>)) != hipSuccess) e = fail(SPP_ERR_HIP, "hipMalloc");
  if (!e && dig.alloc(sizeof(int16_t) * std::max<size_t>(msm_digit_elems((uint32_t)n, 1, cb), 1)) != hipSuccess) e = fail(SPP_ERR_HIP, "hipMalloc");
  XYZZ<F> res = XYZZ<F>::infinity();
  if (!e) {
    launch_msm_digits(st, d_rows, d_sc, dig.as<int16_t>(), (uint32_t)n, 1, cb);
    launch_msm_accumulate<F>(st, table, dig.as<int16_t>(), partial, (uint32_t)n, 1, cb, pl);
    launch_msm_reduce<F>(st, partial, d_out, 1, pl, cb, n == 0);
    if (hipStreamSynchronize(st) != hipSuccess || hipGetLastError() != hipSuccess) e = fail(SPP_ERR_HIP, "msm kernels failed");
    else if (hipMemcpy(&res, d_out, sizeof res, hipMemcpyDeviceToHost) != hipSuccess) e = fail(SPP_ERR_HIP, "copy back failed");
  }
  for (void* p : tmpc.owned) hipFree(p);
  if (partial) hipFree(partial);
  if (d_out) hipFree(d_out);
  if (e) return e;
  point_to_raw(res.to_affine(), out);
  return SPP_OK;
}
extern "C" int spp_msm_g1(spp_ctx* ctx, const uint8_t* bases, const uint8_t* scalars, size_t n, int window_bits, uint8_t out[64]) {
  return msm_fixed_unit<Fq, 64>(ctx, bases, scalars, n, window_bits, out);
}
extern "C" int spp_msm_g2(spp_ctx* ctx, const uint8_t* bases, const uint8_t* scalars, size_t n, int window_bits, uint8_t out[128]) {
  return msm_fixed_unit<Fq2, 128>(ctx, bases, scalars, n, window_bits, out);
}
```

shielded-pool-pinocchio-solana_amd/csrc/spp_plan.cpp:

```cpp
#include "spp_circuit.hpp"

int coop_plan(spp_circuit* c) {
  const Circuit& circ = c->circ;
  const auto& pr = circ.program;
  struct Item { uint32_t kind, a, b; };
  std::vector<uint32_t> items, par, lvl_ptr{0}, lvl_rows, stream;
  const Fr f_one = Fr::one(), f_mone = Fr::one().neg();
  auto coeff_word = [&](uint32_t ci) -> uint32_t {
    return ci | (circ.coeffs[ci] == f_one ? COEFF_ONE : circ.coeffs[ci] == f_mone ? COEFF_MINUS_ONE : 0u);
  };
  auto row_record = [&](uint32_t k, std::vector<uint32_t>& out) {
    const bool square = [&] {
      const uint32_t a0 = circ.A.rowptr[k], a1 = circ.A.rowptr[k + 1], b0 = circ.B.rowptr[k], b1 = circ.B.rowptr[k + 1];
      if (a1 - a0 != b1 - b0) return false;
      for (uint32_t i = 0; i < a1 - a0; i++)
        if (circ.A.terms[a0 + i].wire != circ.B.terms[b0 + i].wire || circ.A.terms[a0 + i].coeff != circ.B.terms[b0 + i].coeff) return false;
      return true;
    }();
    const uint32_t nA = square ? 0 : circ.A.rowptr[k + 1] - circ.A.rowptr[k], nB = circ.B.rowptr[k + 1] - circ.B.rowptr[k],
                   nC = circ.C.rowptr[k + 1] - circ.C.rowptr[k] - 1;
    out.push_back(circ.C.terms[circ.C.rowptr[k + 1] - 1].wire);
    out.push_back(nA | (square ? 0x80000000u : 0u));
    out.push_back(nB);
    out.push_back(nC);
    auto put = [&](const Sparse& m, uint32_t n) {
      for (uint32_t t = m.rowptr[k]; t < m.rowptr[k] + n; t++) { out.push_back(m.terms[t].wire); out.push_back(coeff_word(m.terms[t].coeff)); }
    };
    put(circ.A, nA); put(circ.B, nB); put(circ.C, nC);
  };
  std::vector<uint32_t> level_of(circ.n_wires + 3, 0), stamp(circ.n_wires + 3, 0), writer(circ.n_wires + 3, 0);
  uint32_t epoch = 0;
  auto op_len = [&](size_t pc) -> uint32_t {
    switch (pr[pc]) {
      case OP_SOLVE_C: case OP_SOLVE_A: case OP_MASK: return 2;
      case OP_BATCH_DIV: case OP_POSEIDON2: case OP_INV_H: return 3;
      case OP_COUNT8: case OP_BITS: case OP_LIMBS8: case OP_POSEIDON: return 4;
      case OP_COMMIT: return 1;
      case OP_GRUMPKIN: return 5 + pr[pc + 4];
      default: return 0;
    }
  };
  auto is_par_op = [&](uint32_t op) { return op == OP_BITS || op == OP_LIMBS8 || op == OP_INV_H; };
  struct RW { std::vector<uint32_t> rd, wr; double cost = 0; bool scratch = false; };
  auto row_rd = [&](RW& x, const Sparse& m, uint32_t k, uint32_t skip_last) {
    for (uint32_t t = m.rowptr[k]; t + skip_last < m.rowptr[k + 1]; t++) x.rd.push_back(m.terms[t].wire);
  };
  auto solve_c_rw = [&](RW& x, uint32_t k) {
    row_rd(x, circ.A, k, 0); row_rd(x, circ.B, k, 0); row_rd(x, circ.C, k, 1);
    x.wr.push_back(circ.C.terms[circ.C.rowptr[k + 1] - 1].wire);
  };
  auto div_rw = [&](RW& x, uint32_t k) {
    row_rd(x, circ.B, k, 0); row_rd(x, circ.C, k, 0);
    x.wr.push_back(circ.A.terms[circ.A.rowptr[k]].wire);
  };
  auto op_rw = [&](RW& x, size_t pc, bool coop_form) {
    switch (pr[pc]) {
      case OP_SOLVE_C: solve_c_rw(x, pr[pc + 1]); x.cost += 5; break;
      case OP_SOLVE_A: div_rw(x, pr[pc + 1]); x.cost += 60; x.scratch = true; break;
      case OP_BATCH_DIV:
        for (uint32_t k = 0; k < pr[pc + 2]; k++) div_rw(x, pr[pc + 1] + k);
        x.cost += 60 + 10.0 * pr[pc + 2]; x.scratch = true;
        break;
      case OP_BITS: case OP_LIMBS8:
        row_rd(x, circ.H, pr[pc + 1], 0);
        for (uint32_t i = 0; i < pr[pc + 2]; i++) x.wr.push_back(pr[pc + 3] + i);
        x.cost += 5 + 0.2 * pr[pc + 2];
        break;
      case OP_INV_H: row_rd(x, circ.H, pr[pc + 1], 0); x.wr.push_back(pr[pc + 2]); x.cost += 40; break;
      case OP_MASK: x.wr.push_back(pr[pc + 1]); x.cost += 5; break;
      case OP_POSEIDON: {
        const uint32_t t = pr[pc + 1], nsbox = 8 * t + (t == 3 ? 57 : 60);
        for (uint32_t i = 0; i < t; i++) row_rd(x, circ.H, pr[pc + 2] + i, 0);
        for (uint32_t i = 0; i < 4 * nsbox; i++) x.wr.push_back(pr[pc + 3] + i);
        x.cost += coop_form ? 175 : 450;
        break;
      }
      case OP_POSEIDON2:
        for (uint32_t i = 0; i < 4; i++) row_rd(x, circ.H, pr[pc + 1] + i, 0);
        for (uint32_t i = 0; i < 4 * 88; i++) x.wr.push_back(pr[pc + 2] + i);
        x.cost += coop_form ? 185 : 480;
        break;
      case OP_GRUMPKIN:
        for (uint32_t i = 0; i < pr[pc + 2]; i++) x.rd.push_back(pr[pc + 1] + i);
        for (uint32_t i = 0; i < pr[pc + 4]; i++) x.wr.push_back(pr[pc + 5 + i]);
        x.cost += coop_form ? 300 : 1800;
        x.scratch = x.scratch || !coop_form;
        break;
      default: break;
    }
  };
  for (SolveStep& st : c->schedule) {
    if (st.kind != SolveStep::SEQ) continue;
    std::vector<Item> its;
    size_t pc = st.a, seq0 = st.a;
    auto push = [&](uint32_t kind, uint32_t a, uint32_t b) { its.push_back({kind, a, b}); };
    auto flush = [&](size_t end) {
      if (end > seq0) push(COOP_SEQ, (uint32_t)seq0, (uint32_t)end);
    };
    while (pc < st.b) {
      const uint32_t op = pr[pc];
      if (op == OP_POSEIDON || op == OP_POSEIDON2 || (op == OP_GRUMPKIN && pr[pc + 4] >= 64 && pr[pc + 4] <= 65)) {
        flush(pc);
        push(op == OP_POSEIDON ? COOP_POSEIDON : op == OP_POSEIDON2 ? COOP_POSEIDON2 : COOP_GRUMPKIN, (uint32_t)pc, 0);
        pc += op_len(pc);
        seq0 = pc;
      } else if (op == OP_SOLVE_C) {
        size_t e = pc;
        while (e < st.b && pr[e] == OP_SOLVE_C) e += 2;
        const size_t nrows = (e - pc) / 2;
        if (nrows < 8) { pc = e; continue; }
        flush(pc);
        epoch++;
        std::vector<std::pair<uint32_t, uint32_t>> rows;
        uint32_t max_level = 0;
        for (size_t q = pc; q < e; q += 2) {
          const uint32_t k = pr[q + 1];
          uint32_t lv = 0;
          auto scan = [&](const Sparse& m, uint32_t skip_last) {
            for (uint32_t t = m.rowptr[k]; t + skip_last < m.rowptr[k + 1]; t++) {
              const uint32_t w = m.terms[t].wire;
              if (stamp[w] == epoch) lv = std::max(lv, level_of[w]);
            }
          };
          scan(circ.A, 0); scan(circ.B, 0); scan(circ.C, 1);
          const uint32_t out = circ.C.terms[circ.C.rowptr[k + 1] - 1].wire;
          stamp[out] = epoch;
          level_of[out] = lv + 1;
          rows.push_back({lv, k});
          max_level = std::max(max_level, lv);
        }
        std::vector<uint32_t> rp(rows.size());
        for (size_t i = 0; i < rows.size(); i++) rp[i] = (uint32_t)i;
        auto rfind = [&](uint32_t x) { while (rp[x] != x) x = rp[x] = rp[rp[x]]; return x; };
        epoch++;
        for (size_t i = 0; i < rows.size(); i++) {
          const uint32_t k = rows[i].second;
          auto link = [&](const Sparse& m, uint32_t skip_last) {
            for (uint32_t t = m.rowptr[k]; t + skip_last < m.rowptr[k + 1]; t++) {
              const uint32_t w = m.terms[t].wire;
              if (stamp[w] == epoch) { const uint32_t ra = rfind((uint32_t)i), rb = rfind(writer[w]); if (ra != rb) rp[ra] = rb; }
            }
          };
          link(circ.A, 0); link(circ.B, 0); link(circ.C, 1);
          const uint32_t out = circ.C.terms[circ.C.rowptr[k + 1] - 1].wire;
          stamp[out] = epoch;
          writer[out] = (uint32_t)i;
        }
        std::vector<uint32_t> comp_size(rows.size(), 0), comp_id(rows.size(), 0);
        for (size_t i = 0; i < rows.size(); i++) comp_size[rfind((uint32_t)i)]++;
        const uint32_t MISC = 0xffffffffu;
        std::vector<uint32_t> comp_order;
        bool any_misc = false;
        for (size_t i = 0; i < rows.size(); i++) {
          const uint32_t r = rfind((uint32_t)i);
          if (comp_size[r] < 32) { comp_id[i] = MISC; any_misc = true; continue; }
          comp_id[i] = r;
          if (std::find(comp_order.begin(), comp_order.end(), r) == comp_order.end()) comp_order.push_back(r);
        }
        if (any_misc) comp_order.push_back(MISC);
        std::vector<size_t> order(rows.size());
        for (size_t i = 0; i < rows.size(); i++) order[i] = i;
        std::stable_sort(order.begin(), order.end(), [&](size_t x, size_t y) { return rows[x].first < rows[y].first; });
        for (uint32_t cid : comp_order) {
          const uint32_t l0 = (uint32_t)lvl_ptr.size() - 1;
          uint32_t cur = 0xffffffffu;
          std::vector<std::vector<uint32_t>> by_level;
          for (size_t oi : order) {
            if (comp_id[oi] != cid) continue;
            if (rows[oi].first != cur) {
              if (cur != 0xffffffffu) lvl_ptr.push_back((uint32_t)lvl_rows.size());
              cur = rows[oi].first;
              by_level.emplace_back();
            }
            lvl_rows.push_back(rows[oi].second);
            by_level.back().push_back(rows[oi].second);
          }
          lvl_ptr.push_back((uint32_t)lvl_rows.size());
          std::vector<uint32_t> local;
          uint32_t used = 0;
          bool fits = !c->sw.no_level_stream;
          auto close_chunk = [&] {
            if (used < COOP_CHUNK) local.push_back(0xffffffffu), used++;
            local.resize(local.size() + (COOP_CHUNK - used), 0xffffffffu);
            used = 0;
          };
          for (const auto& lv : by_level) {
            if (!fits) break;
            size_t i = 0;
            while (i < lv.size() && fits) {
              std::vector<std::vector<uint32_t>> recs;
              uint32_t words = 2;
              while (i < lv.size()) {
                std::vector<uint32_t> rec;
                row_record(lv[i], rec);
                if (words + 1 + rec.size() > COOP_CHUNK - 1) break;
                words += 1 + (uint32_t)rec.size();
                recs.push_back(std::move(rec));
                i++;
              }
              if (recs.empty()) { fits = false; break; }
              if (used + words > COOP_CHUNK - 1 && used) close_chunk();
              uint32_t longest = 1;
              for (const auto& rec : recs) longest = std::max({longest, rec[1] & 0x7fffffffu, rec[2], rec[3]});
              uint32_t G = 1;
              while (G < 16 && G < longest && recs.size() * (G * 2) <= 64) G *= 2;
              uint32_t need = 0;
              for (const auto& rec : recs) need |= ((rec[1] & 0x7fffffffu) ? 1u << 29 : 0u) | (rec[3] ? 1u << 30 : 0u);
              local.push_back((uint32_t)recs.size() | (G << 24) | need);
              local.push_back(words);
              uint32_t off = 2 + (uint32_t)recs.size();
              for (const auto& rec : recs) { local.push_back(off); off += (uint32_t)rec.size(); }
              for (const auto& rec : recs) local.insert(local.end(), rec.begin(), rec.end());
              used += words;
            }
          }
          if (fits && !local.empty()) {
            if (used) close_chunk();
            const uint32_t chunk0 = (uint32_t)(stream.size() / COOP_CHUNK);
            stream.insert(stream.end(), local.begin(), local.end());
            push(COOP_LEVEL_STREAM, chunk0, (uint32_t)(local.size() / COOP_CHUNK));
          } else {
            push(COOP_LEVELS, l0, (uint32_t)lvl_ptr.size() - 1);
          }
        }
        pc = e;
        seq0 = pc;
      } else if (is_par_op(op)) {
        size_t e = pc;
        epoch++;
        std::vector<uint32_t> group;
        while (e < st.b && is_par_op(pr[e])) {
          const uint32_t h = pr[e + 1];
          bool dep = false;
          for (uint32_t t = circ.H.rowptr[h]; t < circ.H.rowptr[h + 1]; t++) dep = dep || stamp[circ.H.terms[t].wire] == epoch;
          if (dep) break;
          if (pr[e] == OP_INV_H) stamp[pr[e + 2]] = epoch;
          else for (uint32_t i = 0; i < pr[e + 2]; i++) stamp[pr[e + 3] + i] = epoch;
          group.push_back((uint32_t)e);
          e += op_len(e);
        }
        if (group.size() < 4) { pc = group.empty() ? pc + op_len(pc) : e; continue; }
        flush(pc);
        const uint32_t g0 = (uint32_t)(par.size() / 2);
        for (uint32_t q : group) { par.push_back(q); par.push_back(q + op_len(q)); }
        push(COOP_PAR, g0, g0 + (uint32_t)group.size());
        pc = e;
        seq0 = pc;
      } else {
        const uint32_t n = op_len(pc);
        if (n == 0) return fail(SPP_ERR_FORMAT, "bad opcode %u in solver program", op);
        pc += n;
      }
    }
    flush(st.b);

    const size_t n = its.size();
    std::vector<RW> rw(n);
    for (size_t i = 0; i < n; i++) {
      const Item& it = its[i];
      switch (it.kind) {
        case COOP_SEQ:
          for (size_t q = it.a; q < it.b; q += op_len(q)) op_rw(rw[i], q, false);
          break;
        case COOP_PAR:
          for (uint32_t g = it.a; g < it.b; g++) op_rw(rw[i], par[2 * g], false);
          rw[i].cost = 10 + rw[i].cost / 32;
          break;
        case COOP_LEVELS:
          for (uint32_t r = lvl_ptr[it.a]; r < lvl_ptr[it.b]; r++) solve_c_rw(rw[i], lvl_rows[r]);
          rw[i].cost = 4.5 * (it.b - it.a);
          break;
        case COOP_LEVEL_STREAM: {
          uint32_t nlev = 0;
          for (uint32_t ch = it.a; ch < it.a + it.b; ch++) {
            const uint32_t* sb = stream.data() + (size_t)ch * COOP_CHUNK;
            for (uint32_t pos = 0; pos < COOP_CHUNK && sb[pos] != 0xffffffffu; pos += sb[pos + 1]) {
              nlev++;
              for (uint32_t r = 0; r < (sb[pos] & 0xffffffu); r++) {
                const uint32_t base = pos + sb[pos + 2 + r];
                const uint32_t nt = (sb[base + 1] & 0x7fffffffu) + sb[base + 2] + sb[base + 3];
                rw[i].wr.push_back(sb[base]);
                for (uint32_t t = 0; t < nt; t++) rw[i].rd.push_back(sb[base + 4 + 2 * t]);
              }
            }
          }
          rw[i].cost = 3.0 * nlev;
          break;
        }
        default: op_rw(rw[i], it.a, true); break;
      }
    }
    std::vector<uint32_t> parent(n);
    for (size_t i = 0; i < n; i++) parent[i] = (uint32_t)i;
    auto find = [&](uint32_t x) { while (parent[x] != x) x = parent[x] = parent[parent[x]]; return x; };
    epoch++;
    for (size_t i = 0; i < n; i++) {
      for (uint32_t w : rw[i].rd)
        if (stamp[w] == epoch) { const uint32_t ra = find((uint32_t)i), rb = find(writer[w]); if (ra != rb) parent[ra] = rb; }
      for (uint32_t w : rw[i].wr) { stamp[w] = epoch; writer[w] = (uint32_t)i; }
    }
    std::vector<double> comp_cost(n, 0.0);
    std::vector<char> comp_scratch(n, 0);
    for (size_t i = 0; i < n; i++) { const uint32_t r = find((uint32_t)i); comp_cost[r] += rw[i].cost; comp_scratch[r] |= rw[i].scratch; }
    std::vector<uint32_t> roots;
    for (size_t i = 0; i < n; i++) if (find((uint32_t)i) == i) roots.push_back((uint32_t)i);
    std::sort(roots.begin(), roots.end(), [&](uint32_t x, uint32_t y) { return comp_cost[x] > comp_cost[y]; });
    double load[COOP_TRACKS] = {};
    std::vector<uint32_t> track_of(n, 0);
    for (uint32_t r : roots) if (comp_scratch[r]) { track_of[r] = 0; load[0] += comp_cost[r]; }
    for (uint32_t r : roots) {
      if (comp_scratch[r]) continue;
      uint32_t best = 0;
      for (uint32_t t = 1; t < COOP_TRACKS; t++) if (load[t] < load[best]) best = t;
      track_of[r] = best;
      load[best] += comp_cost[r];
    }
    st.ntracks = 0;
    for (uint32_t t = 0; t < COOP_TRACKS; t++) {
      st.tr_begin[t] = (uint32_t)(items.size() / 3);
      for (size_t i = 0; i < n; i++)
        if (track_of[find((uint32_t)i)] == t) { items.push_back(its[i].kind); items.push_back(its[i].a); items.push_back(its[i].b); }
      st.tr_end[t] = (uint32_t)(items.size() / 3);
      if (st.tr_end[t] > st.tr_begin[t]) st.ntracks = t + 1;
    }
  }
  if (items.empty()) items.assign(3, 0);
  if (par.empty()) par.assign(2, 0);
  if (lvl_rows.empty()) lvl_rows.push_back(0);
  if (stream.empty()) stream.assign(COOP_CHUNK, 0xffffffffu);
  uint32_t *d_items, *d_par, *d_lp, *d_lr, *d_ls;
  int e;
  if ((e = own_upload(c, &d_items, items)) || (e = own_upload(c, &d_par, par)) || (e = own_upload(c, &d_lp, lvl_ptr)) ||
      (e = own_upload(c, &d_lr, lvl_rows)) || (e = own_upload(c, &d_ls, stream)))
    return e;
  c->coop.items = d_items; c->coop.par = d_par; c->coop.lvl_ptr = d_lp; c->coop.lvl_rows = d_lr; c->coop.lvl_stream = d_ls;
  return 0;
}

static constexpr uint32_t SMALL_ROW_MIN = 64, SMALL_ROW_REST = 32;
static int small_rows_plan(spp_circuit* c, std::vector<uint8_t>& flags_out) {
  const Circuit& circ = c->circ;
  c->dc.sm_nrows = 0;
  c->dc.sm_nslots = 0;
  c->dc.row_small = nullptr;
  if (getenv("SPP_NO_SMALL_ROWS")) return 0;
  auto small_of = [&](uint32_t ci, int64_t* out) {
    uint32_t v[8];
    circ.coeffs[ci].to_canonical(v);
    bool hi0 = true;
    for (int k = 1; k < 8; k++) hi0 = hi0 && v[k] == 0;
    if (hi0 && v[0] < (1u << 30)) { *out = (int64_t)v[0]; return true; }
    circ.coeffs[ci].neg().to_canonical(v);
    hi0 = true;
    for (int k = 1; k < 8; k++) hi0 = hi0 && v[k] == 0;
    if (hi0 && v[0] < (1u << 30)) { *out = -(int64_t)v[0]; return true; }
    return false;
  };
  std::vector<int32_t> slot_of(circ.n_wires, -1);
  std::vector<uint32_t> wires{0};
  std::vector<int32_t> lo{0};
  slot_of[0] = 0;
  for (const SolveStep& st : c->schedule) {
    if (st.kind != SolveStep::COUNT8) continue;
    for (uint32_t h = st.a; h < st.a + st.b && h < circ.H.rows(); h++) {
      uint32_t w = 0, nw = 0;
      int64_t cst = 0;
      bool ok = true;
      for (uint32_t t = circ.H.rowptr[h]; t < circ.H.rowptr[h + 1] && ok; t++) {
        const Term& tm = circ.H.terms[t];
        int64_t v;
        if (!small_of(tm.coeff, &v)) { ok = false; break; }
        if (tm.wire == 0) cst += v;
        else if (v == 1) { w = tm.wire; nw++; }
        else ok = false;
      }
      if (!ok || nw != 1 || cst < -32000 || cst > 32000 || slot_of[w] >= 0) continue;
      slot_of[w] = (int32_t)wires.size();
      wires.push_back(w);
      lo.push_back((int32_t)-cst);
    }
  }
  if (wires.size() < 2) return 0;
  std::vector<uint32_t> rowptr{0}, slots, row_out, rest_ptr{0}, rest_wire, rest_coeff;
  std::vector<int32_t> coefs;
  std::vector<uint8_t> flags(std::max<uint32_t>(circ.n_constraints, 1), 0);
  const Sparse* mats[3] = {&circ.A, &circ.B, &circ.C};
  for (uint32_t mi = 0; mi < 3; mi++) {
    const Sparse& m = *mats[mi];
    for (uint32_t k = 0; k < circ.n_constraints; k++) {
      const uint32_t b = m.rowptr[k], e = m.rowptr[k + 1];
      if (e - b < SMALL_ROW_MIN || e - b > (1u << 20)) continue;
      uint32_t n_small = 0;
      for (uint32_t t = b; t < e; t++) {
        int64_t v;
        if (slot_of[m.terms[t].wire] >= 0 && small_of(m.terms[t].coeff, &v)) n_small++;
      }
      if (n_small < SMALL_ROW_MIN || (e - b) - n_small > SMALL_ROW_REST) continue;
      for (uint32_t t = b; t < e; t++) {
        int64_t v = 0;
        if (slot_of[m.terms[t].wire] >= 0 && small_of(m.terms[t].coeff, &v)) {
          slots.push_back((uint32_t)slot_of[m.terms[t].wire]);
          coefs.push_back((int32_t)v);
        } else {
          rest_wire.push_back(m.terms[t].wire);
          rest_coeff.push_back(m.terms[t].coeff);
        }
      }
      rowptr.push_back((uint32_t)slots.size());
      rest_ptr.push_back((uint32_t)rest_wire.size());
      row_out.push_back((mi << 30) | k);
      flags[k] |= (uint8_t)(1u << mi);
    }
  }
  if (row_out.empty()) return 0;
  uint32_t *d_w, *d_rp, *d_sl, *d_ro, *d_xp, *d_xw, *d_xc;
  int32_t *d_lo, *d_co;
  int e;
  if (rest_wire.empty()) { rest_wire.push_back(0); rest_coeff.push_back(0); }
  if ((e = own_upload(c, &d_w, wires)) || (e = own_upload(c, &d_lo, lo)) || (e = own_upload(c, &d_rp, rowptr)) || (e = own_upload(c, &d_sl, slots)) ||
      (e = own_upload(c, &d_co, coefs)) || (e = own_upload(c, &d_ro, row_out)) ||
      (e = own_upload(c, &d_xp, rest_ptr)) || (e = own_upload(c, &d_xw, rest_wire)) || (e = own_upload(c, &d_xc, rest_coeff)))
    return e;
  c->dc.sm_rest_ptr = d_xp; c->dc.sm_rest_wire = d_xw; c->dc.sm_rest_coeff = d_xc;
  c->dc.sm_wires = d_w; c->dc.sm_lo = d_lo; c->dc.sm_nslots = (uint32_t)wires.size();
  c->dc.sm_rowptr = d_rp; c->dc.sm_slot = d_sl; c->dc.sm_coef = d_co; c->dc.sm_row_out = d_ro; c->dc.sm_nrows = (uint32_t)row_out.size();
  flags_out = flags;
  return 0;
}

static constexpr uint32_t LONG_ROW_MIN = 512;
int row_paths_plan(spp_circuit* c) {
  const Circuit& circ = c->circ;
  std::vector<uint8_t> small_flags;
  if (int e = small_rows_plan(c, small_flags)) return e;
  const uint32_t nc = std::max<uint32_t>(circ.n_constraints, 1);
  if (small_flags.empty()) small_flags.assign(nc, 0);
  std::vector<uint8_t> long_flags(nc, 0);
  std::vector<uint32_t> lg;
  c->dc.lg_n = 0;
  c->dc.lg_rows = nullptr;
  c->dc.row_long = nullptr;
  if (!getenv("SPP_NO_LONG_ROWS")) {
    const Sparse* mats[3] = {&circ.A, &circ.B, &circ.C};
    for (uint32_t mi = 0; mi < 3; mi++)
      for (uint32_t k = 0; k < circ.n_constraints; k++)
        if (mats[mi]->rowptr[k + 1] - mats[mi]->rowptr[k] > LONG_ROW_MIN && !(small_flags[k] & (1u << mi))) {
          lg.push_back((mi << 30) | k);
          long_flags[k] |= (uint8_t)(1u << mi);
        }
  }
  int e;
  if (!lg.empty()) {
    uint32_t* d_lg;
    uint8_t* d_lf;
    if ((e = own_upload(c, &d_lg, lg)) || (e = own_upload(c, &d_lf, long_flags))) return e;
    c->dc.lg_rows = d_lg;
    c->dc.lg_n = (uint32_t)lg.size();
    c->dc.row_long = d_lf;
  }
  if (c->dc.sm_nrows) {
    for (uint32_t k = 0; k < nc; k++) small_flags[k] |= long_flags[k];
    uint8_t* d_fl;
    if ((e = own_upload(c, &d_fl, small_flags))) return e;
    c->dc.row_small = d_fl;
  } else {
    c->dc.row_small = c->dc.row_long;
  }
  return 0;
}
```

shielded-pool-pinocchio-solana_amd/csrc/spp_prove.cpp:

```cpp
#include "spp_circuit.hpp"

template <class T>
static int ws_alloc(Workspace& w, T** p, size_t count) {
  HIP_TRY(hipMalloc((void**)p, sizeof(T) * std::max<size_t>(count, 1)));
  w.owned.push_back((void*)*p);
  return 0;
}
template <class F>
static int ws_set(const spp_circuit* c, Workspace& w, const MsmSet<F>* s, MsmBuf<F>* b, size_t P) {
  b->partial_cap = msm_partial_cap(s->N, P, s->c, s->Wt, MsmWalk<F>::waves_per_simd, c->sw.msm);
  int e;
  if ((e = ws_alloc(w, &b->partial, b->partial_cap))) return e;
  return ws_alloc(w, &b->out, P);
}
static int ensure_workspace(spp_circuit* c, Workspace& w, size_t P) {
  if (P <= w.cap) return 0;
  HIP_TRY(hipStreamSynchronize(w.st));
  free_workspace(w);
  int e;
  if ((e = ws_alloc(w, &w.W, (size_t)c->n_rows * P)) || (e = ws_alloc(w, &w.abc, (size_t)3 * c->n * P)) ||
      (e = ws_alloc(w, &w.scratch, (size_t)c->max_batch_div * P)) || (e = ws_alloc(w, &w.commit_affine, P)) ||
      (e = ws_alloc(w, &w.d_inputs, c->in_stride * P)) || (e = ws_alloc(w, &w.d_rs, 64 * P)) ||
      (e = ws_alloc(w, &w.d_proofs, (size_t)SPP_PROOF_LEN * P)) || (e = ws_alloc(w, &w.d_pws, c->pw_stride * P)) ||
      (e = ws_alloc(w, &w.d_status, P)) || (e = ws_alloc(w, &w.counters, 256 * P)))
    return e;
  if ((e = ws_set(c, w, &c->A, &w.A, P)) || (e = ws_set(c, w, &c->B1, &w.B1, P)) || (e = ws_set(c, w, &c->B2, &w.B2, P)) ||
      (e = ws_set(c, w, &c->K, &w.K, P)) || (e = ws_set(c, w, &c->Z, &w.Z, P)) || (e = ws_set(c, w, &c->CB, &w.CB, P)) ||
      (e = ws_set(c, w, &c->CS, &w.CS, P)))
    return e;
  {
    const size_t Ps = std::min<size_t>(P, scaled_blind_max_batch(c->A.N, c->B1.N));
    if ((e = ws_set(c, w, &c->A, &w.sA, Ps)) || (e = ws_set(c, w, &c->B1, &w.rB, Ps)) || (e = ws_alloc(w, &w.Ws, (size_t)c->n_rows * Ps)) ||
        (e = ws_alloc(w, &w.Wr, (size_t)c->n_rows * Ps)))
      return e;
  }
  {
    size_t d1 = 0;
    for (const MsmSet<Fq>* s : {&c->A, &c->B1, &c->K, &c->Z, &c->CB, &c->CS}) d1 = std::max(d1, msm_digit_elems(s->N, (uint32_t)P, s->c));
    w.dig1_cap = d1;
    w.dig2_cap = msm_digit_elems(c->B2.N, (uint32_t)P, c->B2.c);
    if ((e = ws_alloc(w, &w.dig1, w.dig1_cap)) || (e = ws_alloc(w, &w.dig2, w.dig2_cap))) return e;
    if (c->dc.sm_nrows && (e = ws_alloc(w, &w.small, (size_t)c->dc.sm_nslots * P))) return e;
  }
  w.cap = P;
  return 0;
}

static int16_t* ws_dig(Workspace& w, Fq*) { return w.dig1; }
static int16_t* ws_dig(Workspace& w, Fq2*) { return w.dig2; }
template <class F>
static void run_msm(spp_circuit* c, Workspace& w, const MsmSet<F>& s, MsmBuf<F>& b, uint32_t P, bool timed, hipStream_t st_override = nullptr,
                    std::pair<hipEvent_t, hipEvent_t>* ev_override = nullptr, bool fold = true, const Fr* scal_override = nullptr) {
  hipStream_t st = st_override ? st_override : w.st;
  const Fr* scal = scal_override ? scal_override : s.from_h ? w.abc : w.W;
  MsmPlan pl = msm_plan(s.N, P, s.c, s.Wt, MsmWalk<F>::waves_per_simd, c->sw.msm);
  pl.fit(P, b.partial_cap);
  b.plan = pl;
  std::pair<hipEvent_t, hipEvent_t>* ev = nullptr;
  if (timed && w.msm_ev_used < w.msm_ev.size()) ev = &w.msm_ev[w.msm_ev_used++];
  if (ev_override) ev = ev_override;
  int16_t* dig = ws_dig(w, (F*)nullptr);
  launch_msm_digits(st, s.rows, scal, dig, s.N, P, s.c);
  launch_msm_accumulate<F>(st, s.table, dig, b.partial, s.N, P, s.c, pl, ev ? ev->first : nullptr, ev ? ev->second : nullptr);
  if (fold) launch_msm_reduce<F>(st, b.partial, b.out, P, pl, s.c, s.N == 0);
}

static int prove_on_device(spp_circuit* c, Workspace& w, uint32_t P, const uint8_t* d_inputs, const uint8_t* d_rs, uint8_t* d_proofs,
                           uint8_t* d_pws, uint32_t* d_status) {
  hipStream_t st = w.st;
  const Circuit& circ = c->circ;
  const uint32_t n = c->n;
  w.msm_ev_used = 0;
  w.last_P = P;
  const bool scaled_blind = P <= scaled_blind_max_batch(c->A.N, c->B1.N) && !c->sw.no_coop;
  HIP_TRY(hipMemsetAsync(d_status, 0, sizeof(uint32_t) * P, st));
  hipEventRecord(w.ev[0], st);
  launch_load_inputs(st, d_inputs, d_rs, w.W, circ.n_inputs(), circ.n_wires, P);
  hipEventRecord(w.ev_in, st);
  for (const SolveStep& s : c->schedule) {
    switch (s.kind) {
      case SolveStep::SEQ:
        if (P <= c->sw.coop_max_batch && !c->sw.no_coop && c->sw.trace_items) {
          for (uint32_t t = 0; t < s.ntracks; t++)
            for (uint32_t it = s.tr_begin[t]; it < s.tr_end[t]; it++) {
              CoopTracks one{};
              one.n = 1; one.begin[0] = it; one.end[0] = it + 1;
              launch_solve_coop(st, c->dc, c->coop, w.W, w.scratch, one, P);
            }
        } else if (P <= c->sw.coop_max_batch && !c->sw.no_coop) {
          CoopTracks tr{};
          tr.n = c->sw.one_track ? 1 : s.ntracks;
          for (uint32_t t = 0; t < s.ntracks; t++) { tr.begin[t] = s.tr_begin[t]; tr.end[t] = s.tr_end[t]; }
          if (c->sw.one_track) {
            for (uint32_t t = 0; t < s.ntracks; t++) {
              CoopTracks one{};
              one.n = 1; one.begin[0] = s.tr_begin[t]; one.end[0] = s.tr_end[t];
              launch_solve_coop(st, c->dc, c->coop, w.W, w.scratch, one, P);
            }
          } else launch_solve_coop(st, c->dc, c->coop, w.W, w.scratch, tr, P);
        }
        else launch_solve(st, c->dc, w.W, w.scratch, s.a, s.b, P);
        break;
      case SolveStep::BATCH_DIV: launch_batch_div(st, c->dc, w.W, w.scratch, s.a, s.b, P); break;
      case SolveStep::COUNT8: launch_count8(st, c->dc, w.W, w.counters, s.a, s.b, s.c, P); break;
      case SolveStep::COMMIT:
        run_msm(c, w, c->CB, w.CB, P, true);
        launch_challenge(st, w.CB.out, w.W, circ.challenge_wire, P, w.commit_affine, d_status);
        break;
    }
  }
  hipEventRecord(w.ev[1], st);
  hipEventRecord(w.ev_w, st);
  hipStream_t side = (w.st2 != w.st && w.own_st2p && P > c->sw.coop_max_batch) ? w.own_st2p : w.st2;
  if (c->sw.no_side && P <= c->sw.coop_max_batch) side = st;
  hipStreamWaitEvent(side, w.ev_w, 0);
  run_msm(c, w, c->B2, w.B2, P, false, side, &w.g2_ev);
  hipEventRecord(w.ev_b2, side);
  launch_spmv_check(st, c->dc, w.W, w.abc, n, P, d_status, w.small);
  hipEventRecord(w.ev[2], st);
  const size_t bs = (size_t)n * P;
  const uint32_t nt = c->sw.h_mode == 2 ? 2 : 3;
  launch_ntt(st, w.abc, c->logn, P, c->tw_inv, true, nt, bs, c->coset_br);
  launch_ntt(st, w.abc, c->logn, P, c->tw_fwd, false, nt, bs);
  if (c->sw.h_mode == 2) launch_qap_product(st, w.abc, n, P);
  else launch_qap_pointwise(st, w.abc, n, P, c->zinv);
  if (c->sw.h_mode == 0) launch_ntt(st, w.abc, c->logn, P, c->tw_inv, true, 1, bs, c->coset_inv_br);
  hipEventRecord(w.ev[3], st);
  {
    MsmFoldSets<Fq> fs{};
    const MsmSet<Fq>* sets[7] = {&c->A, &c->B1, &c->K, &c->Z, &c->CS, &c->A, &c->B1};
    MsmBuf<Fq>* bufs[7] = {&w.A, &w.B1, &w.K, &w.Z, &w.CS, &w.sA, &w.rB};
    const Fr* scal[7] = {nullptr, nullptr, nullptr, nullptr, nullptr, w.Ws, w.Wr};
    const int nsets = scaled_blind ? 7 : 5;
    if (scaled_blind) launch_scale_witness(st, w.W, w.Ws, w.Wr, c->n_rows, c->row_r, c->row_s, P);
    for (int i = 0; i < nsets; i++) {
      run_msm(c, w, *sets[i], *bufs[i], P, i < 5, nullptr, nullptr, false, scal[i]);
      fs.partial[i] = bufs[i]->partial;
      fs.out[i] = bufs[i]->out;
      fs.Sg[i] = sets[i]->N ? bufs[i]->plan.Sg : 0;
      fs.R[i] = bufs[i]->plan.R;
      fs.c[i] = sets[i]->c;
    }
    launch_msm_reduce_multi<Fq>(st, fs, nsets, P);
  }
  hipEventRecord(w.ev[4], st);
  hipStreamWaitEvent(st, w.ev_b2, 0);
  hipEventRecord(w.ev[5], st);
  AssembleArgs a;
  a.mA = w.A.out; a.mB1 = w.B1.out; a.mB2 = w.B2.out; a.mK = w.K.out; a.mZ = w.Z.out; a.mPok = w.CS.out;
  a.commit_affine = w.commit_affine;
  a.W = w.W; a.row_r = c->row_r; a.row_s = c->row_s; a.n_public = circ.n_public;
  a.sAr = scaled_blind ? w.sA.out : nullptr;
  a.rBs1 = scaled_blind ? w.rB.out : nullptr;
  a.proofs = d_proofs; a.pws = d_pws; a.P = P;
  launch_assemble(st, a);
  hipEventRecord(w.ev[6], st);
  HIP_TRY(hipGetLastError());
  return SPP_OK;
}

static int ws_depth(const spp_circuit* c, size_t count, bool generic_solver) {
  if (c->sw.forced_depth) return c->sw.forced_depth;
  return count <= 256 ? 6 : count <= 768 ? 4 : generic_solver ? 3 : 2;
}
static Workspace& take_workspace(spp_circuit* c, int depth) {
  if (c->next_ws >= depth) c->next_ws = 0;
  const int wi = c->next_ws;
  c->prev_ws = c->last_ws;
  c->last_ws = wi;
  c->next_ws = (wi + 1) % depth;
  return c->ws[wi];
}
static int take_sized_workspace(spp_circuit* c, size_t count, bool generic_solver, Workspace** w) {
  const int depth = ws_depth(c, count, generic_solver);
  *w = &take_workspace(c, depth);
  for (int k = 0; k < depth; k++)
    if (int e = ensure_workspace(c, c->ws[k], count)) return e;
  return 0;
}
static size_t batch_tail(const spp_circuit* c, size_t count) { return count > 64 && !c->sw.no_split ? count % 64 : 0; }
struct BatchIO {
  const uint8_t* rs;
  uint8_t *proofs, *pws;
  uint32_t* status;
  BatchIO at(const spp_circuit* c, size_t off) const {
    return {rs + off * 64, proofs + off * SPP_PROOF_LEN, pws + off * c->pw_stride, status + off};
  }
};
static int prove_on_device(spp_circuit* c, Workspace& w, size_t P, const uint8_t* d_inputs, const BatchIO& io) {
  return prove_on_device(c, w, (uint32_t)P, d_inputs, io.rs, io.proofs, io.pws, io.status);
}

extern "C" int spp_prove_batch_device(spp_circuit* c, size_t count, const void* d_inputs, const void* d_rs, void* d_proofs, void* d_pws,
                                      void* d_status) {
  if (!c || !d_inputs || !d_rs || !d_proofs || !d_pws || !d_status) return fail(SPP_ERR_BAD_INPUT, "NULL argument");
  if (count == 0) return SPP_OK;
  if (count > (1u << 20)) return fail(SPP_ERR_BAD_INPUT, "batch too large");
  std::lock_guard<std::mutex> lk(c->ctx->mu);
  HIP_TRY(hipSetDevice(c->ctx->device));
  Workspace* w;
  if (int e = take_sized_workspace(c, count, c->generic_solver, &w)) return e;
  const BatchIO io{(const uint8_t*)d_rs, (uint8_t*)d_proofs, (uint8_t*)d_pws, (uint32_t*)d_status};
  const size_t tail = batch_tail(c, count), body = count - tail;
  if (int e = prove_on_device(c, *w, body, (const uint8_t*)d_inputs, io)) return e;
  if (!tail) return SPP_OK;
  return prove_on_device(c, c->ws[c->next_ws], tail, (const uint8_t*)d_inputs + body * c->in_stride, io.at(c, body));
}
extern "C" int spp_prove_audit_from_secrets_device(spp_circuit* c, size_t count, const void* d_pk_a, const void* d_pk_b, const void* d_sk,
                                                   const void* d_r, const void* d_e1, const void* d_e2, const void* d_rs, void* d_proofs,
                                                   void* d_pws, void* d_status) {
  if (!c || !d_pk_a || !d_pk_b || !d_sk || !d_r || !d_e1 || !d_e2 || !d_rs || !d_proofs || !d_pws || !d_status)
    return fail(SPP_ERR_BAD_INPUT, "NULL argument");
  if (c->circ.id != SPP_CIRCUIT_AUDIT || c->circ.n_inputs() != 3360) return fail(SPP_ERR_BAD_INPUT, "not the audit circuit");
  if (count == 0) return SPP_OK;
  if (count > (1u << 20)) return fail(SPP_ERR_BAD_INPUT, "batch too large");
  std::lock_guard<std::mutex> lk(c->ctx->mu);
  HIP_TRY(hipSetDevice(c->ctx->device));
  if (int e = spp_ensure_ctx_consts(c->ctx)) return e;
  Workspace* wp;
  if (int e = take_sized_workspace(c, count, false, &wp)) return e;
  Workspace& w = *wp;
  const size_t need = spp_audit_scratch_bytes(count);
  if (need > w.audit_scratch_cap) {
    HIP_TRY(hipStreamSynchronize(w.st));
    if (w.audit_scratch) HIP_TRY(hipFree(w.audit_scratch));
    w.audit_scratch = nullptr;
    w.audit_scratch_cap = 0;
    HIP_TRY(hipMalloc(&w.audit_scratch, need));
    w.audit_scratch_cap = need;
  }
  if (int e = spp_audit_inputs_enqueue(c->ctx, w.st, w.audit_scratch, (const uint32_t*)d_pk_a, (const uint32_t*)d_pk_b, (uint32_t)count,
                                       (const uint8_t*)d_sk, (const int8_t*)d_r, (const int8_t*)d_e1, (const int8_t*)d_e2, w.d_inputs))
    return e;
  return prove_on_device(c, w, count, w.d_inputs, BatchIO{(const uint8_t*)d_rs, (uint8_t*)d_proofs, (uint8_t*)d_pws, (uint32_t*)d_status});
}
static int withdraw_notes_args(spp_circuit* c, spp_merkle_tree* t) {
  if (c->circ.id != SPP_CIRCUIT_WITHDRAW) return fail(SPP_ERR_BAD_INPUT, "not a withdraw circuit");
  if (t->ctx != c->ctx) return fail(SPP_ERR_BAD_INPUT, "the tree belongs to another context");
  if (c->circ.n_inputs() != 10 + t->depth)
    return fail(SPP_ERR_BAD_INPUT, "the circuit takes %u inputs, a withdraw row over a depth-%u tree has %u", c->circ.n_inputs(), t->depth,
                10 + t->depth);
  return SPP_OK;
}
extern "C" int spp_prove_withdraw_notes_device(spp_circuit* c, spp_merkle_tree* t, size_t count, const void* d_notes, const void* d_rs,
                                               void* d_proofs, void* d_pws, void* d_status) {
  if (!c || !t || !d_notes || !d_rs || !d_proofs || !d_pws || !d_status) return fail(SPP_ERR_BAD_INPUT, "NULL argument");
  if (int e = withdraw_notes_args(c, t)) return e;
  if (count == 0) return SPP_OK;
  if (count > (1u << 20)) return fail(SPP_ERR_BAD_INPUT, "batch too large");
  spp_ctx* ctx = c->ctx;
  std::lock_guard<std::mutex> lk(ctx->mu);
  HIP_TRY(hipSetDevice(ctx->device));
  if (int e = spp_ensure_ctx_consts(ctx)) return e;
  Workspace* wp;
  if (int e = take_sized_workspace(c, count, c->generic_solver, &wp)) return e;
  Workspace &w = *wp, &wt = c->ws[c->next_ws];
  const size_t tail = batch_tail(c, count), body = count - tail;
  const uint8_t* notes = (const uint8_t*)d_notes;
  HIP_TRY(hipStreamWaitEvent(ctx->stream, w.ev_in, 0));
  if (tail) HIP_TRY(hipStreamWaitEvent(ctx->stream, wt.ev_in, 0));
  launch_withdraw_rows(ctx->stream, ctx->gk_table, ctx->hc, t->dev, notes, w.d_inputs, (uint32_t)body);
  if (tail) launch_withdraw_rows(ctx->stream, ctx->gk_table, ctx->hc, t->dev, notes + body * SPP_NOTE_LEN, wt.d_inputs, (uint32_t)tail);
  HIP_TRY(hipEventRecord(w.ev_rows, ctx->stream));
  HIP_TRY(hipStreamWaitEvent(w.st, w.ev_rows, 0));
  if (tail) HIP_TRY(hipStreamWaitEvent(wt.st, w.ev_rows, 0));
  const BatchIO io{(const uint8_t*)d_rs, (uint8_t*)d_proofs, (uint8_t*)d_pws, (uint32_t*)d_status};
  if (int e = prove_on_device(c, w, body, w.d_inputs, io)) return e;
  if (!tail) return SPP_OK;
  return prove_on_device(c, wt, tail, wt.d_inputs, io.at(c, body));
}
extern "C" int spp_prove_withdraw_notes(spp_circuit* c, spp_merkle_tree* t, size_t count, const uint8_t* notes, const uint8_t* rs, uint8_t* proofs,
                                        uint8_t* pws, int32_t* status) {
  if (!c || !t || !notes || !proofs || !pws) return fail(SPP_ERR_BAD_INPUT, "NULL argument");
  if (int e = withdraw_notes_args(c, t)) return e;
  if (count == 0) return SPP_OK;
  if (count > (1u << 24)) return fail(SPP_ERR_BAD_INPUT, "too many notes in one call");
  std::vector<uint8_t> rows(count * c->in_stride);
  if (int e = spp_withdraw_rows_from_tree(t, count, notes, rows.data())) return e;
  return spp_prove_batch(c, count, rows.data(), rs, proofs, pws, status);
}
extern "C" int spp_commitment_challenge(spp_circuit* c, size_t count, const uint8_t* inputs, uint8_t* challenges) {
  if (!c || !inputs || !challenges) return fail(SPP_ERR_BAD_INPUT, "NULL argument");
  if (count == 0) return SPP_OK;
  if (count > 4096) return fail(SPP_ERR_BAD_INPUT, "at most 4096 rows per call");
  if (c->CB.N == 0) return fail(SPP_ERR_BAD_INPUT, "the circuit has no commitment");
  std::lock_guard<std::mutex> lk(c->ctx->mu);
  HIP_TRY(hipSetDevice(c->ctx->device));
  Workspace& w = c->ws[c->next_ws];
  if (int e = ensure_workspace(c, w, count)) return e;
  hipStream_t st = w.st;
  const uint32_t P = (uint32_t)count;
  HIP_TRY(hipMemcpyAsync(w.d_inputs, inputs, c->in_stride * count, hipMemcpyHostToDevice, st));
  HIP_TRY(hipMemsetAsync(w.d_rs, 0, 64 * count, st));
  launch_load_inputs(st, w.d_inputs, w.d_rs, w.W, c->circ.n_inputs(), c->circ.n_wires, P);
  for (const SolveStep& s : c->schedule) {
    if (s.kind == SolveStep::COMMIT) break;
    switch (s.kind) {
      case SolveStep::SEQ: launch_solve(st, c->dc, w.W, w.scratch, s.a, s.b, P); break;
      case SolveStep::BATCH_DIV: launch_batch_div(st, c->dc, w.W, w.scratch, s.a, s.b, P); break;
      case SolveStep::COUNT8: launch_count8(st, c->dc, w.W, w.counters, s.a, s.b, s.c, P); break;
      default: break;
    }
  }
  run_msm(c, w, c->CB, w.CB, P, false);
  launch_challenge(st, w.CB.out, w.W, c->circ.challenge_wire, P, w.commit_affine, w.d_status);
  std::vector<Fr> out(count);
  HIP_TRY(hipMemcpyAsync(out.data(), w.W + (size_t)c->circ.challenge_wire * P, sizeof(Fr) * count, hipMemcpyDeviceToHost, st));
  HIP_TRY(hipStreamSynchronize(st));
  for (size_t i = 0; i < count; i++) out[i].to_bytes_be(challenges + 32 * i);
  return SPP_OK;
}
extern "C" int spp_sync(spp_circuit* c) {
  if (!c) return fail(SPP_ERR_BAD_INPUT, "NULL argument");
  HIP_TRY(hipSetDevice(c->ctx->device));
  for (auto& w : c->ws)
    if (w.st) HIP_TRY(hipStreamSynchronize(w.st));
  return SPP_OK;
}
extern "C" int spp_last_timings(spp_circuit* c, float ms[9]) { return spp_timings(c, 0, ms); }
extern "C" int spp_timings(spp_circuit* c, int which, float ms[9]) {
  if (!c || !ms) return fail(SPP_ERR_BAD_INPUT, "NULL argument");
  HIP_TRY(hipSetDevice(c->ctx->device));
  Workspace& w = c->ws[which ? c->prev_ws : c->last_ws];
  if (w.cap == 0) return fail(SPP_ERR_BAD_INPUT, "no such batch");
  HIP_TRY(hipStreamSynchronize(w.st));
  for (int i = 0; i < 6; i++) {
    float t = 0;
    HIP_TRY(hipEventElapsedTime(&t, w.ev[i], w.ev[i + 1]));
    ms[i] = t;
  }
  float tot = 0;
  HIP_TRY(hipEventElapsedTime(&tot, w.ev[0], w.ev[6]));
  ms[6] = tot;
  float sum = 0;
  for (size_t i = 0; i < w.msm_ev_used; i++) {
    float t = 0;
    HIP_TRY(hipEventElapsedTime(&t, w.msm_ev[i].first, w.msm_ev[i].second));
    sum += t;
  }
  ms[7] = w.msm_ev_used ? sum / (float)w.msm_ev_used : 0.f;
  ms[8] = (float)w.msm_ev_used;
  return SPP_OK;
}

extern "C" int spp_msm_kernel_ms(spp_circuit* c, int which, float ms[7]) {
  if (!c || !ms) return fail(SPP_ERR_BAD_INPUT, "NULL argument");
  HIP_TRY(hipSetDevice(c->ctx->device));
  Workspace& w = c->ws[which ? c->prev_ws : c->last_ws];
  if (w.cap == 0) return fail(SPP_ERR_BAD_INPUT, "no such batch");
  HIP_TRY(hipStreamSynchronize(w.st));
  HIP_TRY(hipStreamSynchronize(w.st2));
  if (w.own_st2p) HIP_TRY(hipStreamSynchronize(w.own_st2p));
  for (int i = 0; i < 7; i++) ms[i] = 0.f;
  for (size_t i = 0; i < w.msm_ev_used && i < 6; i++) HIP_TRY(hipEventElapsedTime(&ms[i], w.msm_ev[i].first, w.msm_ev[i].second));
  if (c->B2.N) HIP_TRY(hipEventElapsedTime(&ms[6], w.g2_ev.first, w.g2_ev.second));
  return SPP_OK;
}
extern "C" int spp_set_serial(spp_circuit* c, int on) {
  if (!c) return fail(SPP_ERR_BAD_INPUT, "NULL argument");
  std::lock_guard<std::mutex> lk(c->ctx->mu);
  HIP_TRY(hipSetDevice(c->ctx->device));
  HIP_TRY(hipDeviceSynchronize());
  for (int k = 0; k < SPP_NWS; k++) {
    Workspace& w = c->ws[k];
    w.st = on ? c->ws[0].own_st : w.own_st;
    w.st2 = on ? w.st : w.own_st2;
  }
  return SPP_OK;
}

extern "C" int spp_prove_batch(spp_circuit* c, size_t count, const uint8_t* inputs, const uint8_t* rs, uint8_t* proofs, uint8_t* pws,
                               int32_t* status) {
  if (!c || !inputs || !proofs || !pws) return fail(SPP_ERR_BAD_INPUT, "NULL argument");
  if (count == 0) return SPP_OK;
  std::vector<uint8_t> rnd;
  if (!rs) {
    rnd.resize(64 * count);
    FILE* f = fopen("/dev/urandom", "rb");
    if (!f || fread(rnd.data(), 1, rnd.size(), f) != rnd.size()) {
      if (f) fclose(f);
      return fail(SPP_ERR_IO, "cannot read /dev/urandom");
    }
    fclose(f);
    rs = rnd.data();
  }
  std::vector<uint32_t> st(count);
  {
    std::lock_guard<std::mutex> lk(c->ctx->mu);
    HIP_TRY(hipSetDevice(c->ctx->device));
    const size_t pref = c->circ.n_wires <= 16384 ? 4096 : 2048;
    const size_t chunk = count <= pref + pref / 2 ? count : pref;
    const size_t inl = c->in_stride, pwl = c->pw_stride;
    auto fetch = [&](Workspace& w, size_t off, size_t n) -> int {
      hipStream_t s = w.st;
      HIP_TRY(hipMemcpyAsync(proofs + (size_t)SPP_PROOF_LEN * off, w.d_proofs, (size_t)SPP_PROOF_LEN * n, hipMemcpyDeviceToHost, s));
      HIP_TRY(hipMemcpyAsync(pws + pwl * off, w.d_pws, pwl * n, hipMemcpyDeviceToHost, s));
      HIP_TRY(hipMemcpyAsync(st.data() + off, w.d_status, sizeof(uint32_t) * n, hipMemcpyDeviceToHost, s));
      HIP_TRY(hipStreamSynchronize(s));
      return 0;
    };
    Workspace* prev_w = nullptr;
    size_t prev_off = 0, prev_n = 0;
    std::vector<std::pair<size_t, size_t>> chunks;
    for (size_t off = 0; off < count; off += chunk) {
      const size_t n = std::min(chunk, count - off), t = batch_tail(c, n);
      if (t) {
        chunks.push_back({off, n - t});
        chunks.push_back({off + n - t, t});
      } else chunks.push_back({off, n});
    }
    for (const auto& ch : chunks) {
      const size_t off = ch.first, n = ch.second;
      Workspace& w = take_workspace(c, 2);
      if (int e = ensure_workspace(c, w, n)) return e;
      hipStream_t s = w.st;
      HIP_TRY(hipMemcpyAsync(w.d_inputs, inputs + inl * off, inl * n, hipMemcpyHostToDevice, s));
      HIP_TRY(hipMemcpyAsync(w.d_rs, rs + 64 * off, 64 * n, hipMemcpyHostToDevice, s));
      if (int e = prove_on_device(c, w, (uint32_t)n, w.d_inputs, w.d_rs, w.d_proofs, w.d_pws, w.d_status)) return e;
      if (prev_w)
        if (int e = fetch(*prev_w, prev_off, prev_n)) return e;
      prev_w = &w;
      prev_off = off;
      prev_n = n;
    }
    if (prev_w)
      if (int e = fetch(*prev_w, prev_off, prev_n)) return e;
    for (auto& w : c->ws)
      if (w.st) HIP_TRY(hipStreamSynchronize(w.st));
  }
  int rc = SPP_OK;
  for (size_t i = 0; i < count; i++) {
    int32_t v = st[i] ? SPP_ERR_UNSAT : SPP_OK;
    if (status) status[i] = v;
    if (v && rc == SPP_OK) rc = fail(SPP_ERR_UNSAT, "proof %zu: inputs do not satisfy the circuit", i);
    if (v) memset(proofs + (size_t)SPP_PROOF_LEN * i, 0, SPP_PROOF_LEN);
  }
  return rc;
}

extern "C" int spp_prove_withdraw(spp_circuit* c, const spp_withdraw_inputs* in, const uint8_t rs_seed[64], uint8_t proof[SPP_PROOF_LEN],
                                  uint8_t pw[SPP_WITHDRAW_PW_LEN]) {
  if (!c || !in || !proof || !pw) return fail(SPP_ERR_BAD_INPUT, "NULL argument");
  if (c->circ.id != SPP_CIRCUIT_WITHDRAW) return fail(SPP_ERR_BAD_INPUT, "not a withdraw circuit");
  if (c->circ.n_inputs() != 10 + SPP_TREE_DEPTH) return fail(SPP_ERR_BAD_INPUT, "this entry point serves the depth-16 circuit; use spp_prove_batch");
  std::vector<uint8_t> buf(26 * 32, 0);
  auto put = [&](int i, const uint8_t* v) { memcpy(buf.data() + 32 * i, v, 32); };
  auto put64 = [&](int i, uint64_t v) { for (int k = 0; k < 8; k++) buf[32 * i + 31 - k] = (uint8_t)(v >> (8 * k)); };
  put(0, in->root); put(1, in->nullifier); put(2, in->recipient); put64(3, in->amount); put(4, in->wa_commitment);
  put(5, in->secret_key); put(6, in->owner_x); put(7, in->owner_y); put(8, in->randomness); put64(9, in->index);
  for (int i = 0; i < SPP_TREE_DEPTH; i++) put(10 + i, in->siblings[i]);
  int32_t st = 0;
  return spp_prove_batch(c, 1, buf.data(), rs_seed, proof, pw, &st);
}

extern "C" int spp_debug_witness(spp_circuit* c, uint8_t* out, size_t n_wires) {
  if (!c || !out) return fail(SPP_ERR_BAD_INPUT, "NULL argument");
  std::lock_guard<std::mutex> lk(c->ctx->mu);
  Workspace& w = c->ws[c->last_ws];
  if (w.cap == 0) return fail(SPP_ERR_BAD_INPUT, "no batch has been proved yet");
  HIP_TRY(hipSetDevice(c->ctx->device));
  HIP_TRY(hipStreamSynchronize(w.st));
  size_t P = w.last_P;
  std::vector<Fr> col(std::min<size_t>(n_wires, c->circ.n_wires));
  for (size_t i = 0; i < col.size(); i++) HIP_TRY(hipMemcpy(&col[i], w.W + i * P, sizeof(Fr), hipMemcpyDeviceToHost));
  for (size_t i = 0; i < col.size(); i++) col[i].to_bytes_be(out + 32 * i);
  return SPP_OK;
}
```

Measured before the change: 6647 proofs/s.

## Use ragged per-block MSM tables sized by wire value bounds

The loader now derives value bounds for witness wires (bits, byte limbs, byte-ranged lookups) and builds MSM precompute tables with per-64-row blocks that store only as many multiples as the wire can reach. The walk kernel looks up block offsets and entry counts through a new block descriptor array. The window-size planner counts these narrow bases so the freed table memory can buy wider windows, and fewer windows, for the wide sets. This costs an extra descriptor load per digit and disables the scaled-blind path when A or B1 tables are narrow. Correctness depends on the inferred bounds holding for every witness.

```diff
diff --git a/shielded-pool-pinocchio-solana_amd/csrc/kernels.hpp b/shielded-pool-pinocchio-solana_amd/csrc/kernels.hpp
--- a/shielded-pool-pinocchio-solana_amd/csrc/kernels.hpp
+++ b/shielded-pool-pinocchio-solana_amd/csrc/kernels.hpp
@@ -3,6 +3,7 @@
 #include <stdint.h>
 #include "bn254.hpp"
 #include "msm_plan.hpp"
+#include "msm_ragged.hpp"
 #include "rlwe_ntt.hpp"
 
 namespace spp {
@@ -147,11 +148,11 @@
 };
 template <class F>
 void launch_build_table(hipStream_t st, const Affine<F>* bases, uint32_t N, uint32_t c, uint32_t Wt, uint32_t row0, uint32_t nrows,
-                        Affine<F>* table, XYZZ<F>* tmp, F* tmp_pre);
+                        Affine<F>* table, XYZZ<F>* tmp, F* tmp_pre, const MsmBlock* blocks = nullptr, uint32_t E = 0);
 void launch_msm_digits(hipStream_t st, const uint32_t* rows, const Fr* scalars, int16_t* dig, uint32_t N, uint32_t P, uint32_t c);
 template <class F>
-void launch_msm_accumulate(hipStream_t st, const Affine<F>* table, const int16_t* dig, XYZZ<F>* partial, uint32_t N, uint32_t P, uint32_t c,
-                           const MsmPlan& pl, hipEvent_t ev_start = nullptr, hipEvent_t ev_stop = nullptr);
+void launch_msm_accumulate(hipStream_t st, const Affine<F>* table, const MsmBlock* blocks, const int16_t* dig, XYZZ<F>* partial, uint32_t N, uint32_t P,
+                           uint32_t c, const MsmPlan& pl, hipEvent_t ev_start = nullptr, hipEvent_t ev_stop = nullptr);
 template <class F>
 void launch_msm_reduce(hipStream_t st, XYZZ<F>* partial, XYZZ<F>* out, uint32_t P, const MsmPlan& pl, uint32_t c, bool empty);
 static constexpr uint32_t MSM_FOLD_SETS = 8;
diff --git a/shielded-pool-pinocchio-solana_amd/csrc/kernels_msm.hip b/shielded-pool-pinocchio-solana_amd/csrc/kernels_msm.hip
--- a/shielded-pool-pinocchio-solana_amd/csrc/kernels_msm.hip
+++ b/shielded-pool-pinocchio-solana_amd/csrc/kernels_msm.hip
@@ -3,9 +3,9 @@
 namespace spp {
 
 template void launch_build_table<Fq>(hipStream_t, const Affine<Fq>*, uint32_t, uint32_t, uint32_t, uint32_t, uint32_t, Affine<Fq>*,
-                                     XYZZ<Fq>*, Fq*);
-template void launch_msm_accumulate<Fq>(hipStream_t, const Affine<Fq>*, const int16_t*, XYZZ<Fq>*, uint32_t, uint32_t, uint32_t, const MsmPlan&,
-                                        hipEvent_t, hipEvent_t);
+                                     XYZZ<Fq>*, Fq*, const MsmBlock*, uint32_t);
+template void launch_msm_accumulate<Fq>(hipStream_t, const Affine<Fq>*, const MsmBlock*, const int16_t*, XYZZ<Fq>*, uint32_t, uint32_t, uint32_t,
+                                        const MsmPlan&, hipEvent_t, hipEvent_t);
 template void launch_msm_reduce_multi<Fq>(hipStream_t, MsmFoldSets<Fq>, uint32_t, uint32_t);
 template void launch_msm_reduce<Fq>(hipStream_t, XYZZ<Fq>*, XYZZ<Fq>*, uint32_t, const MsmPlan&, uint32_t, bool);
 template void launch_fixed_base_mul<Fq>(hipStream_t, const Affine<Fq>*, uint32_t, const Fr*, uint32_t, Affine<Fq>*);
diff --git a/shielded-pool-pinocchio-solana_amd/csrc/kernels_msm_g2.hip b/shielded-pool-pinocchio-solana_amd/csrc/kernels_msm_g2.hip
--- a/shielded-pool-pinocchio-solana_amd/csrc/kernels_msm_g2.hip
+++ b/shielded-pool-pinocchio-solana_amd/csrc/kernels_msm_g2.hip
@@ -3,9 +3,9 @@
 namespace spp {
 
 template void launch_build_table<Fq2>(hipStream_t, const Affine<Fq2>*, uint32_t, uint32_t, uint32_t, uint32_t, uint32_t, Affine<Fq2>*,
-                                      XYZZ<Fq2>*, Fq2*);
-template void launch_msm_accumulate<Fq2>(hipStream_t, const Affine<Fq2>*, const int16_t*, XYZZ<Fq2>*, uint32_t, uint32_t, uint32_t,
-                                         const MsmPlan&, hipEvent_t, hipEvent_t);
+                                     XYZZ<Fq2>*, Fq2*, const MsmBlock*, uint32_t);
+template void launch_msm_accumulate<Fq2>(hipStream_t, const Affine<Fq2>*, const MsmBlock*, const int16_t*, XYZZ<Fq2>*, uint32_t, uint32_t, uint32_t,
+                                        const MsmPlan&, hipEvent_t, hipEvent_t);
 template void launch_msm_reduce_multi<Fq2>(hipStream_t, MsmFoldSets<Fq2>, uint32_t, uint32_t);
 template void launch_msm_reduce<Fq2>(hipStream_t, XYZZ<Fq2>*, XYZZ<Fq2>*, uint32_t, const MsmPlan&, uint32_t, bool);
 template void launch_fixed_base_mul<Fq2>(hipStream_t, const Affine<Fq2>*, uint32_t, const Fr*, uint32_t, Affine<Fq2>*);
diff --git a/shielded-pool-pinocchio-solana_amd/csrc/msm_classes.hpp b/shielded-pool-pinocchio-solana_amd/csrc/msm_classes.hpp
--- /dev/null
+++ b/shielded-pool-pinocchio-solana_amd/csrc/msm_classes.hpp
@@ -0,0 +1,78 @@
+#pragma once
+#include "circuit.hpp"
+#include "msm_ragged.hpp"
+
+namespace spp {
+
+inline bool fr_small_signed(const Fr& x, int64_t* out) {
+  uint32_t v[8];
+  x.to_canonical(v);
+  bool hi0 = true;
+  for (int k = 1; k < 8; k++) hi0 = hi0 && v[k] == 0;
+  if (hi0 && v[0] < (1u << 30)) { *out = (int64_t)v[0]; return true; }
+  x.neg().to_canonical(v);
+  hi0 = true;
+  for (int k = 1; k < 8; k++) hi0 = hi0 && v[k] == 0;
+  if (hi0 && v[0] < (1u << 30)) { *out = -(int64_t)v[0]; return true; }
+  return false;
+}
+inline bool circuit_byte_ranged_lookup(const Circuit& circ, uint32_t h, uint32_t* wire, int64_t* cst) {
+  if (h >= circ.H.rows()) return false;
+  const Term* t = circ.H.terms.data();
+  return byte_ranged_lookup(t + circ.H.rowptr[h], t + circ.H.rowptr[h + 1], [&](uint32_t ci, int64_t* v) { return fr_small_signed(circ.coeffs[ci], v); },
+                            wire, cst);
+}
+
+enum : uint8_t { WIRE_WIDE = 0, WIRE_BIT = 1, WIRE_LIMB8 = 2, WIRE_LOOKUP = 3 };
+struct WireClasses {
+  std::vector<uint32_t> bound;
+  std::vector<uint8_t> kind;
+};
+inline WireClasses msm_wire_classes(const Circuit& circ) {
+  WireClasses wc;
+  wc.bound.assign(circ.n_wires, 0);
+  wc.kind.assign(circ.n_wires, WIRE_WIDE);
+  auto mark = [&](uint32_t w, uint32_t b, uint8_t kind) {
+    if (w == 0 || w >= circ.n_wires) return;
+    if (wc.kind[w] == WIRE_WIDE) wc.kind[w] = kind;
+    narrow_wire(wc.bound, w, b);
+  };
+  const std::vector<uint32_t>& pr = circ.program;
+  auto all_wide = [&]() {
+    wc.bound.assign(circ.n_wires, 0);
+    wc.kind.assign(circ.n_wires, WIRE_WIDE);
+    return wc;
+  };
+  for (size_t pc = 0; pc < pr.size() && pr[pc] != OP_END;) {
+    size_t len = 0;
+    switch (pr[pc]) {
+      case OP_SOLVE_C: case OP_SOLVE_A: case OP_MASK: len = 2; break;
+      case OP_BATCH_DIV: case OP_POSEIDON2: case OP_INV_H: len = 3; break;
+      case OP_COUNT8: case OP_BITS: case OP_LIMBS8: case OP_POSEIDON: len = 4; break;
+      case OP_COMMIT: len = 1; break;
+      case OP_GRUMPKIN: len = pc + 4 < pr.size() ? 5 + (size_t)pr[pc + 4] : 0; break;
+      default: return all_wide();
+    }
+    if (len == 0 || pc + len > pr.size()) return all_wide();
+    if (pr[pc] == OP_BITS)
+      for (uint32_t i = 0; i < pr[pc + 2]; i++) mark(pr[pc + 3] + i, 1, WIRE_BIT);
+    if (pr[pc] == OP_LIMBS8)
+      for (uint32_t i = 0; i < pr[pc + 2]; i++) mark(pr[pc + 3] + i, 255, WIRE_LIMB8);
+    if (pr[pc] == OP_COUNT8)
+      for (uint32_t i = 0; i < pr[pc + 2]; i++) {
+        uint32_t w;
+        int64_t cst;
+        if (circuit_byte_ranged_lookup(circ, pr[pc + 1] + i, &w, &cst)) mark(w, byte_ranged_bound(cst), WIRE_LOOKUP);
+      }
+    pc += len;
+  }
+  return wc;
+}
+inline std::vector<uint32_t> msm_base_bounds(const WireClasses& wc, const std::vector<uint32_t>& rows) {
+  std::vector<uint32_t> b(rows.size(), 0);
+  for (size_t i = 0; i < rows.size(); i++)
+    if (rows[i] < wc.bound.size()) b[i] = wc.bound[rows[i]];
+  return b;
+}
+
+}
diff --git a/shielded-pool-pinocchio-solana_amd/csrc/msm_ragged.hpp b/shielded-pool-pinocchio-solana_amd/csrc/msm_ragged.hpp
--- /dev/null
+++ b/shielded-pool-pinocchio-solana_amd/csrc/msm_ragged.hpp
@@ -0,0 +1,123 @@
+#pragma once
+#include <stddef.h>
+#include <stdint.h>
+
+#include <algorithm>
+#include <numeric>
+#include <vector>
+
+#include "msm_plan.hpp"
+
+namespace spp {
+
+
+template <class TermIt, class SmallOf>
+inline bool byte_ranged_lookup(TermIt begin, TermIt end, SmallOf small, uint32_t* wire, int64_t* cst_out) {
+  uint32_t w = 0, nw = 0;
+  int64_t cst = 0;
+  for (TermIt t = begin; t != end; ++t) {
+    int64_t v;
+    if (!small(t->coeff, &v)) return false;
+    if (t->wire == 0) cst += v;
+    else if (v == 1) { w = t->wire; nw++; }
+    else return false;
+  }
+  if (nw != 1 || cst < -32000 || cst > 32000) return false;
+  *wire = w;
+  *cst_out = cst;
+  return true;
+}
+inline uint32_t byte_ranged_bound(int64_t cst) {
+  const int64_t lo = cst < 0 ? -cst : cst, hi = 255 - cst < 0 ? cst - 255 : 255 - cst;
+  return (uint32_t)std::max<int64_t>(std::max(lo, hi), 1);
+}
+inline void narrow_wire(std::vector<uint32_t>& bound, uint32_t wire, uint32_t b) {
+  if (wire == 0 || wire >= bound.size()) return;
+  if (bound[wire] == 0 || b < bound[wire]) bound[wire] = b;
+}
+
+struct MsmBlock {
+  uint64_t off;
+  uint32_t E;
+  uint32_t pad_;
+};
+inline uint32_t msm_class_entries(uint32_t bound, uint32_t c) {
+  const uint32_t full = 1u << (c - 1);
+  if (bound == 0 || bound >= full) return full;
+  uint32_t e = 1;
+  while (e < bound) e <<= 1;
+  return e;
+}
+struct MsmRagged {
+  std::vector<MsmBlock> blocks;
+  uint64_t units = 0;
+  size_t elems() const { return (size_t)units * 64; }
+  size_t index(size_t row, uint32_t d) const { return (size_t)(blocks[row >> 6].off + d) * 64 + (row & 63); }
+  bool narrow(uint32_t c) const {
+    for (const MsmBlock& b : blocks) if (b.E != (1u << (c - 1))) return true;
+    return false;
+  }
+};
+inline MsmRagged msm_ragged_layout(const uint32_t* bound, size_t N, uint32_t c) {
+  MsmRagged L;
+  const size_t nb = (N + 63) / 64;
+  L.blocks.resize(nb);
+  for (size_t b = 0; b < nb; b++) {
+    uint32_t E = 1;
+    for (size_t r = b * 64; r < std::min(N, b * 64 + 64); r++) E = std::max(E, msm_class_entries(bound[r], c));
+    L.blocks[b] = {L.units, E, 0};
+    L.units += E;
+  }
+  return L;
+}
+inline std::vector<uint32_t> msm_class_major_order(const uint32_t* bound, size_t N, uint32_t c) {
+  std::vector<uint32_t> perm(N);
+  std::iota(perm.begin(), perm.end(), 0u);
+  std::stable_sort(perm.begin(), perm.end(), [&](uint32_t a, uint32_t b) { return msm_class_entries(bound[a], c) > msm_class_entries(bound[b], c); });
+  return perm;
+}
+
+struct PlanSet {
+  double n, esz, wgt;
+  bool flat;
+  int bits;
+  double narrow[3] = {0, 0, 0};
+};
+static constexpr double PLAN_NARROW_E[3] = {1, 128, 256};
+inline double plan_wide(const PlanSet& s) { return s.flat ? s.n - s.narrow[0] - s.narrow[1] - s.narrow[2] : s.n; }
+inline double plan_bytes(const PlanSet& s, int cb) {
+  const double full = (double)(1u << (cb - 1));
+  if (!s.flat) return s.n * s.esz * (double)msm_windows((uint32_t)cb) * full;
+  double rows = plan_wide(s) * full;
+  for (int k = 0; k < 3; k++) rows += s.narrow[k] * std::min(PLAN_NARROW_E[k], full);
+  return rows * s.esz;
+}
+inline void plan_greedy(std::vector<PlanSet>& sets, double budget, int cmax) {
+  double used = 0;
+  for (auto& s : sets) used += plan_bytes(s, s.bits);
+  for (;;) {
+    int best = -1;
+    double best_gain = 0;
+    for (size_t i = 0; i < sets.size(); i++) {
+      const PlanSet& s = sets[i];
+      if (s.wgt == 0 || s.bits >= cmax || s.n == 0) continue;
+      const double extra = plan_bytes(s, s.bits + 1) - plan_bytes(s, s.bits);
+      if (used + extra > budget) continue;
+      const double saved = s.wgt * plan_wide(s) * ((double)msm_windows((uint32_t)s.bits) - (double)msm_windows((uint32_t)s.bits + 1));
+      double gain = saved / extra;
+      if (saved <= 0) gain = 1e-30;
+      if (gain > best_gain) { best_gain = gain; best = (int)i; }
+    }
+    if (best < 0) break;
+    used += plan_bytes(sets[best], sets[best].bits + 1) - plan_bytes(sets[best], sets[best].bits);
+    sets[best].bits++;
+  }
+}
+static constexpr double PLAN_ESZ[7] = {64, 64, 64, 64, 64, 64, 128}, PLAN_WGT[7] = {1, 1, 1, 1, 0, 0, 3.0};
+inline PlanSet plan_set(int s, double n, bool flat) { return {n, PLAN_ESZ[s], PLAN_WGT[s], flat, PLAN_WGT[s] != 0 ? 6 : 9}; }
+inline void plan_count(PlanSet& s, uint32_t bound) {
+  if (bound == 0 || bound > 256) return;
+  s.narrow[bound <= 1 ? 0 : bound <= 128 ? 1 : 2] += 1;
+}
+
+}
diff --git a/shielded-pool-pinocchio-solana_amd/csrc/msm_table.hpp b/shielded-pool-pinocchio-solana_amd/csrc/msm_table.hpp
--- a/shielded-pool-pinocchio-solana_amd/csrc/msm_table.hpp
+++ b/shielded-pool-pinocchio-solana_amd/csrc/msm_table.hpp
@@ -10,14 +10,14 @@
 static constexpr unsigned MSM_WALK_BLOCK = 64;
 
 template <class F>
-__global__ void __launch_bounds__(64) k_build_table(const Affine<F>* __restrict__ bases, uint32_t N, uint32_t c, uint32_t Wn,
+__global__ void __launch_bounds__(64) k_build_table(const Affine<F>* __restrict__ bases, uint32_t N, uint32_t E, uint32_t Wn,
                                                     uint32_t step_bits, uint32_t row0, uint32_t nrows, Affine<F>* __restrict__ table,
-                                                    XYZZ<F>* __restrict__ tmp, F* __restrict__ tmp_pre) {
+                                                    XYZZ<F>* __restrict__ tmp, F* __restrict__ tmp_pre, const MsmBlock* __restrict__ blocks) {
   const uint32_t rl = blockIdx.x * blockDim.x + threadIdx.x;
   if (rl >= nrows) return;
   const uint32_t row = row0 + rl;
-  const uint32_t E = 1u << (c - 1);
-  Affine<F>* out = table + ((size_t)(row >> 6) * E) * 64 + (row & 63);
+  const size_t off = blocks ? (size_t)blocks[row >> 6].off : (size_t)(row >> 6) * E;
+  Affine<F>* out = table + off * 64 + (row & 63);
   XYZZ<F>* t = tmp + rl;
   F* pre = tmp_pre + rl;
   if (row >= N * Wn) {
@@ -53,12 +53,13 @@
 }
 template <class F>
 void launch_build_table(hipStream_t st, const Affine<F>* bases, uint32_t N, uint32_t c, uint32_t Wt, uint32_t row0, uint32_t nrows,
-                        Affine<F>* table, XYZZ<F>* tmp, F* tmp_pre) {
+                        Affine<F>* table, XYZZ<F>* tmp, F* tmp_pre, const MsmBlock* blocks, uint32_t E) {
   if (nrows == 0) return;
   const uint32_t W = msm_windows(c);
   if (Wt == 0 || Wt > W) Wt = W;
   const uint32_t R = (W + Wt - 1) / Wt;
-  hipLaunchKernelGGL(k_build_table<F>, dim3((nrows + 63) / 64), dim3(64), 0, st, bases, N, c, Wt, c * R, row0, nrows, table, tmp, tmp_pre);
+  if (!blocks) E = 1u << (c - 1);
+  hipLaunchKernelGGL(k_build_table<F>, dim3((nrows + 63) / 64), dim3(64), 0, st, bases, N, E, Wt, c * R, row0, nrows, table, tmp, tmp_pre, blocks);
 }
 
 struct Recoder {
@@ -124,14 +125,13 @@
 
 
 template <class F>
-__global__ void __launch_bounds__(MSM_WALK_BLOCK, MsmWalk<F>::waves_per_simd) k_msm_flat(const Affine<F>* __restrict__ table, const int16_t* __restrict__ dig,
-                                                  XYZZ<F>* __restrict__ partial, uint32_t N, uint32_t P, uint32_t Pp, uint32_t c,
-                                                  uint32_t R, uint32_t Sg) {
+__global__ void __launch_bounds__(MSM_WALK_BLOCK, MsmWalk<F>::waves_per_simd) k_msm_flat(const Affine<F>* __restrict__ table, const MsmBlock* __restrict__ blocks,
+                                                  const int16_t* __restrict__ dig, XYZZ<F>* __restrict__ partial, uint32_t N, uint32_t P,
+                                                  uint32_t Pp, uint32_t R, uint32_t Sg) {
   const uint32_t g = blockIdx.x * blockDim.x + threadIdx.x;
   const uint32_t p = g % Pp, t = g / Pp;
   if (t >= R * Sg || p >= P) return;
   const uint32_t rho = t / Sg, sl = t % Sg;
-  const uint32_t E = 1u << (c - 1);
   const int16_t* __restrict__ dg = dig + ((size_t)rho * N) * Pp + p;
   MsmAcc<F> acc;
   acc.init();
@@ -150,15 +150,16 @@
       }
 #pragma unroll 1
       for (uint32_t k = 0; k < 4; k++) {
-        const int d = (int)(int16_t)(uint16_t)(pack >> (16 * k));
+        int d = (int)(int16_t)(uint16_t)(pack >> (16 * k));
         const bool flush = last && k == 0;
+        const uint32_t i = i0 + k * Sg;
+        const uint32_t mag = (uint32_t)(d < 0 ? -d : d);
+        MsmBlock blk{};
+        if (d != 0) blk = blocks[i >> 6];
+        if (mag > blk.E) d = 0;
         if (d != 0 || flush) {
           Affine<F> e;
-          if (d != 0) {
-            const uint32_t i = i0 + k * Sg;
-            const uint32_t mag = (uint32_t)(d < 0 ? -d : d);
-            e = table[((size_t)(i >> 6) * E + (mag - 1)) * 64 + (i & 63)];
-          }
+          if (d != 0) e = table[((size_t)blk.off + (mag - 1)) * 64 + (i & 63)];
           if (d_next != 0) acc.madd(e_next, d_next < 0);
           d_next = d;
           if (d != 0) e_next = e;
@@ -181,7 +182,8 @@
         if (d != 0) {
           const uint32_t i = i0 + k * Sg;
           const uint32_t mag = (uint32_t)(d < 0 ? -d : d);
-          acc.madd(table[((size_t)(i >> 6) * E + (mag - 1)) * 64 + (i & 63)], d < 0);
+          const MsmBlock blk = blocks[i >> 6];
+          if (mag <= blk.E) acc.madd(table[((size_t)blk.off + (mag - 1)) * 64 + (i & 63)], d < 0);
         }
       }
     }
@@ -226,8 +228,8 @@
 }
 
 template <class F>
-void launch_msm_accumulate(hipStream_t st, const Affine<F>* table, const int16_t* dig, XYZZ<F>* partial, uint32_t N, uint32_t P, uint32_t c,
-                           const MsmPlan& pl, hipEvent_t ev_start, hipEvent_t ev_stop) {
+void launch_msm_accumulate(hipStream_t st, const Affine<F>* table, const MsmBlock* blocks, const int16_t* dig, XYZZ<F>* partial, uint32_t N, uint32_t P,
+                           uint32_t c, const MsmPlan& pl, hipEvent_t ev_start, hipEvent_t ev_stop) {
   if (N == 0 || P == 0) {
     if (ev_start) hipEventRecord(ev_start, st);
     if (ev_stop) hipEventRecord(ev_stop, st);
@@ -235,7 +237,7 @@
   }
   const uint64_t lanes = (uint64_t)pl.R * pl.Sg * pl.Pp;
   if (pl.Wt == 1)
-    hipExtLaunchKernelGGL(k_msm_flat<F>, dim3((uint32_t)((lanes + MSM_WALK_BLOCK - 1) / MSM_WALK_BLOCK)), dim3(MSM_WALK_BLOCK), 0, st, ev_start, ev_stop, 0, table, dig, partial, N, P, pl.Pp, c, pl.R, pl.Sg);
+    hipExtLaunchKernelGGL(k_msm_flat<F>, dim3((uint32_t)((lanes + MSM_WALK_BLOCK - 1) / MSM_WALK_BLOCK)), dim3(MSM_WALK_BLOCK), 0, st, ev_start, ev_stop, 0, table, blocks, dig, partial, N, P, pl.Pp, pl.R, pl.Sg);
   else
     hipExtLaunchKernelGGL(k_msm_rows<F>, dim3((uint32_t)((lanes + 255) / 256)), dim3(256), 0, st, ev_start, ev_stop, 0, table, dig, partial, N, P, pl.Pp, c,
                           pl.Wt, pl.R, pl.W, pl.Sg, pl.Q, pl.Wq);
diff --git a/shielded-pool-pinocchio-solana_amd/csrc/spp_circuit.hpp b/shielded-pool-pinocchio-solana_amd/csrc/spp_circuit.hpp
--- a/shielded-pool-pinocchio-solana_amd/csrc/spp_circuit.hpp
+++ b/shielded-pool-pinocchio-solana_amd/csrc/spp_circuit.hpp
@@ -1,5 +1,6 @@
 #pragma once
 #include "spp_internal.hpp"
+#include "msm_classes.hpp"
 
 template <class F>
 struct MsmSet {
@@ -9,6 +10,8 @@
   bool from_h = false;
   uint32_t c = 0;
   uint32_t Wt = 0;
+  MsmBlock* blocks = nullptr;
+  bool narrow = false;
 };
 template <class F>
 struct MsmBuf {
@@ -51,6 +54,8 @@
   std::vector<Affine<F>> pts;
   Affine<F>* table;
   uint32_t c, Wt;
+  MsmRagged layout;
+  const MsmBlock* blocks;
 };
 struct SolveStep {
   enum Kind { SEQ, BATCH_DIV, COUNT8, COMMIT } kind;
@@ -67,6 +72,7 @@
   bool no_side = false;
   int forced_depth = 0;
   bool no_split = false;
+  bool ragged = true;
   MsmTuning msm;
 };
 static constexpr uint64_t SCALED_BLIND_MAX_SCALARS = 1500000;
diff --git a/shielded-pool-pinocchio-solana_amd/csrc/spp_load.cpp b/shielded-pool-pinocchio-solana_amd/csrc/spp_load.cpp
--- a/shielded-pool-pinocchio-solana_amd/csrc/spp_load.cpp
+++ b/shielded-pool-pinocchio-solana_amd/csrc/spp_load.cpp
@@ -40,8 +40,8 @@
 }
 
 template <class F>
-static int alloc_table(spp_circuit* c, size_t N, uint32_t cbits, uint32_t Wt, Affine<F>** table_out) {
-  size_t table_elems = std::max<size_t>(msm_table_elems((uint32_t)N, cbits, Wt), 1);
+static int alloc_table_elems(spp_circuit* c, size_t table_elems, Affine<F>** table_out) {
+  table_elems = std::max<size_t>(table_elems, 1);
   Affine<F>* table;
   HIP_TRY(hipMalloc((void**)&table, table_elems * sizeof(Affine<F>)));
   c->owned.push_back(table);
@@ -50,24 +50,40 @@
   return 0;
 }
 template <class F>
-static int build_table(spp_circuit* c, const std::vector<Affine<F>>& pts, uint32_t cbits, uint32_t Wt, Affine<F>* table, size_t temp_budget) {
+static int alloc_table(spp_circuit* c, size_t N, uint32_t cbits, uint32_t Wt, Affine<F>** table_out) {
+  return alloc_table_elems<F>(c, msm_table_elems((uint32_t)N, cbits, Wt), table_out);
+}
+template <class F>
+static int build_table(spp_circuit* c, const std::vector<Affine<F>>& pts, uint32_t cbits, uint32_t Wt, Affine<F>* table, size_t temp_budget,
+                       const MsmRagged* layout = nullptr, const MsmBlock* blocks = nullptr) {
   hipStream_t st = c->ctx->stream;
-  const uint32_t Wn = Wt, E = 1u << (cbits - 1);
+  const uint32_t Wn = Wt, Efull = 1u << (cbits - 1);
   const size_t N = pts.size();
   if (N == 0) return 0;
+  if (!layout || layout->blocks.empty()) { layout = nullptr; blocks = nullptr; }
   const size_t rows_total = msm_table_rows(N, Wn);
-  const size_t per_row = (size_t)E * (sizeof(XYZZ<F>) + sizeof(F));
+  uint32_t Emax = layout ? 1 : Efull;
+  if (layout) for (const MsmBlock& b : layout->blocks) Emax = std::max(Emax, b.E);
+  const size_t per_row = (size_t)Emax * (sizeof(XYZZ<F>) + sizeof(F));
   size_t chunk = std::max<size_t>(64, ((temp_budget / per_row) / 64) * 64);
   chunk = std::min(chunk, (size_t)65536);
   chunk = std::min(chunk, rows_total);
   DevBuf d_bases, tmp, tmp_pre;
   HIP_TRY(d_bases.alloc(N * sizeof(Affine<F>)));
   HIP_TRY(hipMemcpy(d_bases.p, pts.data(), N * sizeof(Affine<F>), hipMemcpyHostToDevice));
-  HIP_TRY(tmp.alloc(chunk * E * sizeof(XYZZ<F>)));
-  HIP_TRY(tmp_pre.alloc(chunk * E * sizeof(F)));
-  for (size_t r0 = 0; r0 < rows_total; r0 += chunk) {
-    uint32_t cnt = (uint32_t)std::min(chunk, rows_total - r0);
-    launch_build_table<F>(st, d_bases.as<Affine<F>>(), (uint32_t)N, cbits, Wt, (uint32_t)r0, cnt, table, tmp.as<XYZZ<F>>(), tmp_pre.as<F>());
+  HIP_TRY(tmp.alloc(chunk * Emax * sizeof(XYZZ<F>)));
+  HIP_TRY(tmp_pre.alloc(chunk * Emax * sizeof(F)));
+  for (size_t r0 = 0; r0 < rows_total;) {
+    size_t r1 = rows_total;
+    uint32_t E = Efull;
+    if (layout) {
+      E = layout->blocks[r0 >> 6].E;
+      r1 = r0 + 64;
+      while (r1 < rows_total && layout->blocks[r1 >> 6].E == E) r1 += 64;
+    }
+    uint32_t cnt = (uint32_t)std::min(chunk, r1 - r0);
+    launch_build_table<F>(st, d_bases.as<Affine<F>>(), (uint32_t)N, cbits, Wt, (uint32_t)r0, cnt, table, tmp.as<XYZZ<F>>(), tmp_pre.as<F>(), blocks, E);
+    r0 += cnt;
   }
   HIP_TRY(hipStreamSynchronize(st));
   HIP_TRY(hipGetLastError());
@@ -88,22 +104,43 @@
 
 
 template <class F>
-static int make_set(spp_circuit* c, MsmSet<F>* set, const std::vector<uint32_t>& rows, const std::vector<Affine<F>>& pts, bool from_h,
-                    uint32_t cbits, bool flat) {
+static int make_set(spp_circuit* c, MsmSet<F>* set, std::vector<uint32_t> rows, std::vector<Affine<F>> pts, bool from_h, uint32_t cbits,
+                    bool flat, std::vector<uint32_t> bound = {}) {
   set->N = (uint32_t)pts.size();
   set->from_h = from_h;
   set->c = cbits;
   set->Wt = flat ? 1 : msm_windows(cbits);
-  if (int e = own_upload(c, &set->rows, rows)) return e;
-  if (int e = alloc_table<F>(c, pts.size(), cbits, set->Wt, &set->table)) return e;
-  pending(c, (F*)nullptr).push_back({pts, set->table, cbits, set->Wt});
+  if (!flat) {
+    if (int e = own_upload(c, &set->rows, rows)) return e;
+    if (int e = alloc_table<F>(c, pts.size(), cbits, set->Wt, &set->table)) return e;
+    pending(c, (F*)nullptr).push_back({std::move(pts), set->table, cbits, set->Wt, MsmRagged{}, nullptr});
+    return 0;
+  }
+  bound.resize(pts.size(), 0);
+  if (!c->sw.ragged) std::fill(bound.begin(), bound.end(), 0u);
+  const std::vector<uint32_t> perm = msm_class_major_order(bound.data(), bound.size(), cbits);
+  std::vector<uint32_t> rows_o(perm.size()), bound_o(perm.size());
+  std::vector<Affine<F>> pts_o(perm.size());
+  for (size_t k = 0; k < perm.size(); k++) {
+    rows_o[k] = rows[perm[k]];
+    pts_o[k] = pts[perm[k]];
+    bound_o[k] = bound[perm[k]];
+  }
+  MsmRagged layout = msm_ragged_layout(bound_o.data(), bound_o.size(), cbits);
+  set->narrow = layout.narrow(cbits);
+  if (int e = own_upload(c, &set->rows, rows_o)) return e;
+  if (layout.blocks.empty()) layout.blocks.push_back({0, 1u << (cbits - 1), 0});
+  if (int e = own_upload(c, &set->blocks, layout.blocks)) return e;
+  if (int e = alloc_table_elems<F>(c, layout.elems(), &set->table)) return e;
+  if (pts_o.empty()) layout.blocks.clear();
+  pending(c, (F*)nullptr).push_back({std::move(pts_o), set->table, cbits, set->Wt, std::move(layout), set->blocks});
   return 0;
 }
 static int build_pending(spp_circuit* c) {
   const size_t budget = table_temp_budget();
   int e = 0;
-  for (auto& p : pending(c, (Fq*)nullptr)) if (!e) e = build_table<Fq>(c, p.pts, p.c, p.Wt, p.table, budget);
-  for (auto& p : pending(c, (Fq2*)nullptr)) if (!e) e = build_table<Fq2>(c, p.pts, p.c, p.Wt, p.table, budget);
+  for (auto& p : pending(c, (Fq*)nullptr)) if (!e) e = build_table<Fq>(c, p.pts, p.c, p.Wt, p.table, budget, &p.layout, p.blocks);
+  for (auto& p : pending(c, (Fq2*)nullptr)) if (!e) e = build_table<Fq2>(c, p.pts, p.c, p.Wt, p.table, budget, &p.layout, p.blocks);
   pending(c, (Fq*)nullptr).clear();
   pending(c, (Fq2*)nullptr).clear();
   return e;
@@ -191,40 +228,10 @@
   pts.push_back(extra);
 }
 
-namespace {
-struct PlanSet {
-  double n, esz, wgt;
-  bool flat;
-  int bits;
-};
-double plan_bytes(const PlanSet& s, int cb) { return s.n * s.esz * (s.flat ? 1.0 : (double)msm_windows((uint32_t)cb)) * (double)(1u << (cb - 1)); }
-void plan_greedy(std::vector<PlanSet>& sets, double budget, int cmax) {
-  double used = 0;
-  for (auto& s : sets) used += plan_bytes(s, s.bits);
-  for (;;) {
-    int best = -1;
-    double best_gain = 0;
-    for (size_t i = 0; i < sets.size(); i++) {
-      const PlanSet& s = sets[i];
-      if (s.wgt == 0 || s.bits >= cmax || s.n == 0) continue;
-      const double extra = plan_bytes(s, s.bits + 1) - plan_bytes(s, s.bits);
-      if (used + extra > budget) continue;
-      const double saved = s.wgt * s.n * ((double)msm_windows((uint32_t)s.bits) - (double)msm_windows((uint32_t)s.bits + 1));
-      double gain = saved / extra;
-      if (saved <= 0) gain = 1e-30;
-      if (gain > best_gain) { best_gain = gain; best = (int)i; }
-    }
-    if (best < 0) break;
-    used += plan_bytes(sets[best], sets[best].bits + 1) - plan_bytes(sets[best], sets[best].bits);
-    sets[best].bits++;
-  }
-}
-const double PLAN_ESZ[7] = {64, 64, 64, 64, 64, 64, 128}, PLAN_WGT[7] = {1, 1, 1, 1, 0, 0, 3.0};
-}
-
 struct LoadState {
   PkFile pk;
   uint32_t cw[7];
+  WireClasses wc;
   bool flat[7] = {false, false, false, false, false, false, false};
   std::vector<uint32_t> z_w, xk_w;
   std::vector<G1Affine> z_p, xk_p;
@@ -245,11 +252,13 @@
   const int depth = de ? atoi(de) : 0;
   sw.forced_depth = depth >= 1 && depth <= SPP_NWS ? depth : 0;
   sw.no_split = getenv("SPP_NO_SPLIT") != nullptr;
+  const char* rg = getenv("SPP_RAGGED");
+  sw.ragged = !(rg && rg[0] == '0');
   sw.msm = msm_tuning_from_env(getenv("SPP_MSM_WAVES"), getenv("SPP_MSM_WAVES_SMALL"));
   return sw;
 }
 
-static int plan_load_windows(const PkFile& pk, int window_bits, const uint32_t* forced_bits, uint32_t cw[7], bool flat[7]) {
+static int plan_load_windows(const PkFile& pk, const WireClasses& wc, int window_bits, const uint32_t* forced_bits, uint32_t cw[7], bool flat[7]) {
   const double nset[7] = {(double)pk.A.size() + 2, (double)pk.B1.size() + 2, (double)pk.K.size() + 1, (double)pk.Z.size(),
                           (double)pk.CB.size(), (double)pk.CS.size(), (double)pk.B2.size() + 2};
   if (forced_bits) {
@@ -270,8 +279,12 @@
     std::vector<PlanSet> sets;
     for (int s = 0; s < 7; s++) {
       flat[s] = use_flat && PLAN_WGT[s] != 0;
-      sets.push_back({nset[s], PLAN_ESZ[s], PLAN_WGT[s], flat[s], PLAN_WGT[s] != 0 ? 6 : 9});
-    }
+      sets.push_back(plan_set(s, nset[s], flat[s]));
+    }
+    const std::vector<uint32_t>* keyed[7] = {&pk.A_w, &pk.B1_w, &pk.K_w, nullptr, nullptr, nullptr, &pk.B2_w};
+    for (int s = 0; s < 7; s++)
+      if (keyed[s] && flat[s])
+        for (uint32_t b : msm_base_bounds(wc, *keyed[s])) plan_count(sets[s], b);
     plan_greedy(sets, budget, use_flat ? 16 : 15);
     for (int s = 0; s < 7; s++) cw[s] = (uint32_t)sets[s].bits;
   }
@@ -480,21 +493,21 @@
     std::vector<G1Affine> p = pk.A;
     merge_point(w, p, 0u, pk.alpha1);
     w.push_back(c->row_r); p.push_back(pk.delta1);
-    if ((e = make_set(c, &c->A, w, p, false, cw[0], flat[0]))) return e;
+    if ((e = make_set(c, &c->A, w, p, false, cw[0], flat[0], msm_base_bounds(s.wc, w)))) return e;
   }
   {
     std::vector<uint32_t> w = pk.B1_w;
     std::vector<G1Affine> p = pk.B1;
     merge_point(w, p, 0u, pk.beta1);
     w.push_back(c->row_s); p.push_back(pk.delta1);
-    if ((e = make_set(c, &c->B1, w, p, false, cw[1], flat[1]))) return e;
+    if ((e = make_set(c, &c->B1, w, p, false, cw[1], flat[1], msm_base_bounds(s.wc, w)))) return e;
   }
   {
     std::vector<uint32_t> w = pk.B2_w;
     std::vector<G2Affine> p = pk.B2;
     merge_point(w, p, 0u, pk.beta2);
     w.push_back(c->row_s); p.push_back(pk.delta2);
-    if ((e = make_set(c, &c->B2, w, p, false, cw[6], flat[6]))) return e;
+    if ((e = make_set(c, &c->B2, w, p, false, cw[6], flat[6], msm_base_bounds(s.wc, w)))) return e;
   }
   return 0;
 }
@@ -612,7 +625,8 @@
       }
     }
     w.push_back(c->row_rs); p.push_back(pk.delta1.neg());
-    if ((e = make_set(c, &c->K, w, p, false, cw[2], flat[2]))) return e;
+    std::vector<uint32_t> kb = msm_base_bounds(s.wc, pk.K_w);
+    if ((e = make_set(c, &c->K, w, p, false, cw[2], flat[2], kb))) return e;
   }
   if ((e = make_set(c, &c->Z, z_w, z_p, true, cw[3], flat[3]))) return e;
   if ((e = make_set(c, &c->CB, pk.CB_w, pk.CB, false, cw[4], false))) return e;
@@ -675,7 +689,9 @@
   if (pk.circuit_id != circ.id || pk.n_wires != circ.n_wires || pk.domain_log != circ.domain_log)
     return fail(SPP_ERR_FORMAT, "proving key does not match the circuit");
   c->sw = read_switches();
-  if (int e = plan_load_windows(pk, window_bits, forced_bits, s.cw, s.flat)) return e;
+  s.wc = msm_wire_classes(circ);
+  if (!c->sw.ragged) s.wc = WireClasses{std::vector<uint32_t>(circ.n_wires, 0), std::vector<uint8_t>(circ.n_wires, WIRE_WIDE)};
+  if (int e = plan_load_windows(pk, s.wc, window_bits, forced_bits, s.cw, s.flat)) return e;
   c->c_bits = s.cw[3];
   c->logn = circ.domain_log;
   c->n = 1u << c->logn;
@@ -780,7 +796,7 @@
   if (!sizes || !bits || n_circuits == 0 || n_circuits > 16) return fail(SPP_ERR_BAD_INPUT, "bad argument");
   std::vector<PlanSet> sets;
   for (uint32_t k = 0; k < n_circuits; k++)
-    for (int s = 0; s < 7; s++) sets.push_back({(double)sizes[7 * k + s], PLAN_ESZ[s], PLAN_WGT[s], PLAN_WGT[s] != 0, PLAN_WGT[s] != 0 ? 6 : 9});
+    for (int s = 0; s < 7; s++) sets.push_back(plan_set(s, (double)sizes[7 * k + s], PLAN_WGT[s] != 0));
   double floor_bytes = 0;
   for (auto& ps : sets) floor_bytes += plan_bytes(ps, ps.bits);
   if (floor_bytes > budget_bytes) return fail(SPP_ERR_BAD_INPUT, "the budget does not hold even 6-bit tables (%.1f GB needed)", floor_bytes / 1e9);
@@ -829,7 +845,7 @@
   XYZZ<F> res = XYZZ<F>::infinity();
   if (!e) {
     launch_msm_digits(st, d_rows, d_sc, dig.as<int16_t>(), (uint32_t)n, 1, cb);
-    launch_msm_accumulate<F>(st, table, dig.as<int16_t>(), partial, (uint32_t)n, 1, cb, pl);
+    launch_msm_accumulate<F>(st, table, nullptr, dig.as<int16_t>(), partial, (uint32_t)n, 1, cb, pl);
     launch_msm_reduce<F>(st, partial, d_out, 1, pl, cb, n == 0);
     if (hipStreamSynchronize(st) != hipSuccess || hipGetLastError() != hipSuccess) e = fail(SPP_ERR_HIP, "msm kernels failed");
     else if (hipMemcpy(&res, d_out, sizeof res, hipMemcpyDeviceToHost) != hipSuccess) e = fail(SPP_ERR_HIP, "copy back failed");
diff --git a/shielded-pool-pinocchio-solana_amd/csrc/spp_plan.cpp b/shielded-pool-pinocchio-solana_amd/csrc/spp_plan.cpp
--- a/shielded-pool-pinocchio-solana_amd/csrc/spp_plan.cpp
+++ b/shielded-pool-pinocchio-solana_amd/csrc/spp_plan.cpp
@@ -344,18 +344,7 @@
   c->dc.sm_nslots = 0;
   c->dc.row_small = nullptr;
   if (getenv("SPP_NO_SMALL_ROWS")) return 0;
-  auto small_of = [&](uint32_t ci, int64_t* out) {
-    uint32_t v[8];
-    circ.coeffs[ci].to_canonical(v);
-    bool hi0 = true;
-    for (int k = 1; k < 8; k++) hi0 = hi0 && v[k] == 0;
-    if (hi0 && v[0] < (1u << 30)) { *out = (int64_t)v[0]; return true; }
-    circ.coeffs[ci].neg().to_canonical(v);
-    hi0 = true;
-    for (int k = 1; k < 8; k++) hi0 = hi0 && v[k] == 0;
-    if (hi0 && v[0] < (1u << 30)) { *out = -(int64_t)v[0]; return true; }
-    return false;
-  };
+  auto small_of = [&](uint32_t ci, int64_t* out) { return fr_small_signed(circ.coeffs[ci], out); };
   std::vector<int32_t> slot_of(circ.n_wires, -1);
   std::vector<uint32_t> wires{0};
   std::vector<int32_t> lo{0};
@@ -363,18 +352,9 @@
   for (const SolveStep& st : c->schedule) {
     if (st.kind != SolveStep::COUNT8) continue;
     for (uint32_t h = st.a; h < st.a + st.b && h < circ.H.rows(); h++) {
-      uint32_t w = 0, nw = 0;
+      uint32_t w = 0;
       int64_t cst = 0;
-      bool ok = true;
-      for (uint32_t t = circ.H.rowptr[h]; t < circ.H.rowptr[h + 1] && ok; t++) {
-        const Term& tm = circ.H.terms[t];
-        int64_t v;
-        if (!small_of(tm.coeff, &v)) { ok = false; break; }
-        if (tm.wire == 0) cst += v;
-        else if (v == 1) { w = tm.wire; nw++; }
-        else ok = false;
-      }
-      if (!ok || nw != 1 || cst < -32000 || cst > 32000 || slot_of[w] >= 0) continue;
+      if (!circuit_byte_ranged_lookup(circ, h, &w, &cst) || slot_of[w] >= 0) continue;
       slot_of[w] = (int32_t)wires.size();
       wires.push_back(w);
       lo.push_back((int32_t)-cst);
diff --git a/shielded-pool-pinocchio-solana_amd/csrc/spp_prove.cpp b/shielded-pool-pinocchio-solana_amd/csrc/spp_prove.cpp
--- a/shielded-pool-pinocchio-solana_amd/csrc/spp_prove.cpp
+++ b/shielded-pool-pinocchio-solana_amd/csrc/spp_prove.cpp
@@ -61,7 +61,7 @@
   if (ev_override) ev = ev_override;
   int16_t* dig = ws_dig(w, (F*)nullptr);
   launch_msm_digits(st, s.rows, scal, dig, s.N, P, s.c);
-  launch_msm_accumulate<F>(st, s.table, dig, b.partial, s.N, P, s.c, pl, ev ? ev->first : nullptr, ev ? ev->second : nullptr);
+  launch_msm_accumulate<F>(st, s.table, s.blocks, dig, b.partial, s.N, P, s.c, pl, ev ? ev->first : nullptr, ev ? ev->second : nullptr);
   if (fold) launch_msm_reduce<F>(st, b.partial, b.out, P, pl, s.c, s.N == 0);
 }
 
@@ -72,7 +72,7 @@
   const uint32_t n = c->n;
   w.msm_ev_used = 0;
   w.last_P = P;
-  const bool scaled_blind = P <= scaled_blind_max_batch(c->A.N, c->B1.N) && !c->sw.no_coop;
+  const bool scaled_blind = P <= scaled_blind_max_batch(c->A.N, c->B1.N) && !c->sw.no_coop && !c->A.narrow && !c->B1.narrow;
   HIP_TRY(hipMemsetAsync(d_status, 0, sizeof(uint32_t) * P, st));
   hipEventRecord(w.ev[0], st);
   launch_load_inputs(st, d_inputs, d_rs, w.W, circ.n_inputs(), circ.n_wires, P);
```

Measured after the change: 6792 proofs/s, median of 6. +2.2%, better.
